# MecatronicaUSB/uwimageproc

Hardware: NVIDIA B200
Metric: chain_frames_per_s_4k (higher is better)
Workload: dtype u8 (histretch, aclahe) / int32+f64 (bgdehaze)

## Files before the change

### include/uwip.h

```cpp
#ifndef UWIP_H
#define UWIP_H

#include <stddef.h>
#include <stdint.h>

#ifdef __cplusplus
extern "C" {
#endif

#define UWIP_VERSION 100

typedef enum uwip_status {
  UWIP_OK = 0,
  UWIP_ERR_INVALID = -1,
  UWIP_ERR_CUDA = -2,
  UWIP_ERR_UNSUPPORTED = -3,
  UWIP_ERR_NOMEM = -4
} uwip_status;

typedef enum uwip_hsv_round {
  UWIP_HSV_ROUND_CV2_4_13 = 0,
  UWIP_HSV_ROUND_TRUNC = 1,
  UWIP_HSV_ROUND_RINT = 2
} uwip_hsv_round;

typedef enum uwip_order {
  UWIP_ORDER_INTENDED = 0,
  UWIP_ORDER_LITERAL = 1
} uwip_order;

typedef struct uwip_ctx uwip_ctx;

int uwip_version(void);
int uwip_create(int device, uwip_ctx** out);
void uwip_destroy(uwip_ctx* ctx);
const char* uwip_last_error(const uwip_ctx* ctx);
int uwip_set_stream(uwip_ctx* ctx, void* cuda_stream);
int uwip_synchronize(uwip_ctx* ctx);
int64_t uwip_launch_count(const uwip_ctx* ctx);
int uwip_profile(uwip_ctx* ctx, int enable);
int uwip_profile_read(uwip_ctx* ctx, const char* tag, double* total_ms, int64_t* launches);

int uwip_device_alloc(uwip_ctx* ctx, size_t bytes, void** dptr);
int uwip_device_free(uwip_ctx* ctx, void* dptr);
int uwip_host_alloc(uwip_ctx* ctx, size_t bytes, void** hptr);
int uwip_host_free(uwip_ctx* ctx, void* hptr);
int uwip_copy_h2d(uwip_ctx* ctx, void* dst_dev, const void* src_host, size_t bytes);
int uwip_copy_d2h(uwip_ctx* ctx, void* dst_host, const void* src_dev, size_t bytes);

int uwip_num_channel(char c);
int uwip_num_space(char c);
int uwip_histogram_u8(uwip_ctx* ctx, const uint8_t* plane, int width, int height, size_t pitch,
                      float hist[256]);
int uwip_histogram_u8_dev(uwip_ctx* ctx, const uint8_t* d_plane, int width, int height,
                          float* d_hist);
int uwip_channel_stretch_u8(uwip_ctx* ctx, const uint8_t* src, size_t src_pitch, uint8_t* dst,
                            size_t dst_pitch, int width, int height, int lo, int hi, int* low_bin,
                            int* high_bin);
int uwip_channel_stretch_u8_dev(uwip_ctx* ctx, const uint8_t* d_src, uint8_t* d_dst, int width,
                                int height, int lo, int hi);
int uwip_channel_stretch_u8_dev_pitched(uwip_ctx* ctx, const uint8_t* d_src, size_t src_pitch,
                                        uint8_t* d_dst, size_t dst_pitch, int width, int height, int lo,
                                        int hi);

int uwip_histretch_bgr8(uwip_ctx* ctx, const uint8_t* src, size_t src_pitch, uint8_t* dst,
                        size_t dst_pitch, int width, int height, const char* channels, int lo,
                        int hi, int order, int hsv_round);
int uwip_histretch_bgr8_dev(uwip_ctx* ctx, const uint8_t* d_src, uint8_t* d_dst, int n_frames,
                            int width, int height, const char* channels, int lo, int hi, int order,
                            int hsv_round);

int uwip_clahe_u8(uwip_ctx* ctx, const uint8_t* src, size_t src_pitch, uint8_t* dst,
                  size_t dst_pitch, int width, int height, double clip, int tiles_x, int tiles_y);
int uwip_clahe_u8_dev(uwip_ctx* ctx, const uint8_t* d_src, uint8_t* d_dst, int n_planes, int width,
                      int height, double clip, int tiles_x, int tiles_y);
int uwip_entropy_u8(uwip_ctx* ctx, const uint8_t* plane, int width, int height, size_t pitch,
                    int flavour, float* entropy);
int uwip_gaussian_blur3_u8(uwip_ctx* ctx, const uint8_t* src, size_t src_pitch, uint8_t* dst,
                           size_t dst_pitch, int width, int height);
int uwip_clahe_entropy_sweep_u8(uwip_ctx* ctx, const uint8_t* plane, int width, int height,
                                size_t pitch, int tiles, const double* clips, int n_clips,
                                int flavour, float* entropies);
int uwip_clahe_entropy_sweep_u8_dev(uwip_ctx* ctx, const uint8_t* d_planes, int n_frames, int width, int height,
                                    const int* grids, int n_grids, const double* clips, int n_clips,
                                    int flavour, float* entropies);
int uwip_aclahe_bgr8(uwip_ctx* ctx, const uint8_t* src, size_t src_pitch, uint8_t* dst,
                     size_t dst_pitch, int width, int height, double clip, int tiles_x,
                     int tiles_y, int hsv_round);
int uwip_aclahe_bgr8_dev(uwip_ctx* ctx, const uint8_t* d_src, uint8_t* d_dst, int n_frames,
                         int width, int height, double clip, int tiles_x, int tiles_y,
                         int hsv_round);

typedef enum uwip_aclahe_loop {
  UWIP_ACLAHE_LOOP_REPAIRED = 0,
  UWIP_ACLAHE_LOOP_AS_COMMITTED = 1
} uwip_aclahe_loop;
int uwip_aclahe_params_u8_dev(uwip_ctx* ctx, const uint8_t* d_planes, int n_planes, int width, int height, int loop,
                              int32_t* d_bs, int32_t* d_cl);
int uwip_aclahe_bgr8_auto_dev(uwip_ctx* ctx, const uint8_t* d_src, uint8_t* d_dst, int n_frames, int width, int height,
                              int loop, int hsv_round, double clip, int tiles_x, int tiles_y, int32_t* d_bs,
                              int32_t* d_cl);

typedef struct uwip_dehaze_params {
  int window;
  int radius;
  double eps;
  double tmin;
} uwip_dehaze_params;
void uwip_dehaze_defaults(uwip_dehaze_params* p);

int uwip_boxfilter_f64(uwip_ctx* ctx, const double* src, int width, int height, int r, double* dst);
int uwip_guided_filter_u8(uwip_ctx* ctx, const uint8_t* guide, size_t pitch, int width, int height,
                          int range, const double* p, int r, double eps, double* q);
int uwip_background_light_bgr8(uwip_ctx* ctx, const uint8_t* src, size_t pitch, int width,
                               int height, int window, double B[3], int64_t idx[2]);
int uwip_transmission_bgr8(uwip_ctx* ctx, const uint8_t* src, size_t pitch, int width, int height,
                           int window, double* t_blue, double* t_green);
int uwip_refined_transmission_bgr8(uwip_ctx* ctx, const uint8_t* src, size_t pitch, int width,
                                   int height, const uwip_dehaze_params* p, double* t_blue,
                                   double* t_green);
int uwip_rc_correction_bgr8(uwip_ctx* ctx, const uint8_t* src, size_t pitch, int width, int height,
                            const uwip_dehaze_params* p, double* restored);
int uwip_bgdehaze_bgr8(uwip_ctx* ctx, const uint8_t* src, size_t src_pitch, uint8_t* dst8,
                       size_t dst_pitch, int width, int height, const uwip_dehaze_params* p,
                       double* out_f64);
int uwip_bgdehaze_bgr8_dev(uwip_ctx* ctx, const uint8_t* d_src, uint8_t* d_dst, int n_frames,
                           int width, int height, const uwip_dehaze_params* p);

typedef struct uwip_chain_params {
  char channels[16];
  int lo, hi;
  int order;
  int hsv_round;
  double clip;
  int tiles_x, tiles_y;
  uwip_dehaze_params dehaze;
} uwip_chain_params;
void uwip_chain_defaults(uwip_chain_params* p);

int uwip_chain_bgr8_dev(uwip_ctx* ctx, const uint8_t* d_src, uint8_t* d_dst, int n_frames,
                        int width, int height, const uwip_chain_params* p);
int uwip_chain_bgr8_auto_dev(uwip_ctx* ctx, const uint8_t* d_src, uint8_t* d_dst, int n_frames, int width, int height,
                             const uwip_chain_params* p, int loop, int32_t* d_bs, int32_t* d_cl);
int uwip_chain_bgr8(uwip_ctx* ctx, const uint8_t* src, uint8_t* dst, int n_frames, int width,
                    int height, const uwip_chain_params* p);

#define UWIP_FRAME_NAN 1
#define UWIP_FRAME_ACLAHE_NOFIT 2
int uwip_last_frame_flags(uwip_ctx* ctx, int n_frames, int32_t* flags_host);

int uwip_calc_blur_bgr8(uwip_ctx* ctx, const uint8_t* src, size_t pitch, int width, int height,
                        int aperture, float* stdev, double* mean_std, uint8_t* lap, size_t lap_pitch);
int uwip_calc_blur_bgr8_dev(uwip_ctx* ctx, const uint8_t* d_src, int n_frames, int width, int height,
                            int aperture, double* d_mean_std);

int uwip_jpeg_info(uwip_ctx* ctx, const uint8_t* jpeg, size_t len, int* width, int* height);
int uwip_jpeg_decode_bgr8_dev(uwip_ctx* ctx, const uint8_t* jpeg, size_t len, uint8_t* d_bgr, int width,
                              int height);
int uwip_jpeg_encode_bgr8_dev(uwip_ctx* ctx, const uint8_t* d_bgr, int width, int height, int quality,
                              uint8_t* out, size_t cap, size_t* out_len);
int uwip_chain_jpeg(uwip_ctx* ctx, const uint8_t* jpeg_in, size_t len_in, const uwip_chain_params* p,
                    int quality, uint8_t* jpeg_out, size_t cap, size_t* len_out);
size_t uwip_jpeg_encode_bound(int width, int height);
int uwip_jpeg_encode_bgr8_batch_dev(uwip_ctx* ctx, const uint8_t* d_bgr, int n_frames, int width, int height, int quality,
                                    uint8_t* d_out, size_t out_stride, uint64_t* d_len);

int uwip_synth_bgr8_dev(uwip_ctx* ctx, uint8_t* d_dst, uint32_t seed, int first_frame, int n_frames,
                        int width, int height);
int uwip_checksum_bgr8_dev(uwip_ctx* ctx, const uint8_t* d_src, int n_frames, int width, int height,
                           uint64_t* sums_host);

#ifdef __cplusplus
}
#endif
#endif
```

### uwimageproc_b200/_lib.py

```python
import ctypes as C
import os

HERE = os.path.dirname(os.path.abspath(__file__))
LIB_PATH = os.path.join(HERE, "libuwip.so")

UWIP_OK = 0


class UwipError(RuntimeError):
    def __init__(self, status, text):
        super().__init__("uwip status %d: %s" % (status, text))
        self.status = status


class DehazeParams(C.Structure):
    _fields_ = [("window", C.c_int), ("radius", C.c_int), ("eps", C.c_double), ("tmin", C.c_double)]


class ChainParams(C.Structure):
    _fields_ = [
        ("channels", C.c_char * 16),
        ("lo", C.c_int), ("hi", C.c_int), ("order", C.c_int), ("hsv_round", C.c_int),
        ("clip", C.c_double), ("tiles_x", C.c_int), ("tiles_y", C.c_int),
        ("dehaze", DehazeParams),
    ]


_P = C.c_void_p
_u8p = C.c_void_p
_sz = C.c_size_t
_i = C.c_int
_d = C.c_double

SIGNATURES = {
    "uwip_version": (_i, []),
    "uwip_create": (_i, [_i, C.POINTER(_P)]),
    "uwip_destroy": (None, [_P]),
    "uwip_last_error": (C.c_char_p, [_P]),
    "uwip_set_stream": (_i, [_P, _P]),
    "uwip_synchronize": (_i, [_P]),
    "uwip_launch_count": (C.c_int64, [_P]),
    "uwip_profile": (_i, [_P, _i]),
    "uwip_profile_read": (_i, [_P, C.c_char_p, C.POINTER(_d), C.POINTER(C.c_int64)]),
    "uwip_device_alloc": (_i, [_P, _sz, C.POINTER(_P)]),
    "uwip_device_free": (_i, [_P, _P]),
    "uwip_host_alloc": (_i, [_P, _sz, C.POINTER(_P)]),
    "uwip_host_free": (_i, [_P, _P]),
    "uwip_copy_h2d": (_i, [_P, _P, _P, _sz]),
    "uwip_copy_d2h": (_i, [_P, _P, _P, _sz]),
    "uwip_num_channel": (_i, [C.c_char]),
    "uwip_num_space": (_i, [C.c_char]),
    "uwip_histogram_u8": (_i, [_P, _u8p, _i, _i, _sz, _P]),
    "uwip_histogram_u8_dev": (_i, [_P, _u8p, _i, _i, _P]),
    "uwip_channel_stretch_u8": (_i, [_P, _u8p, _sz, _u8p, _sz, _i, _i, _i, _i, C.POINTER(_i), C.POINTER(_i)]),
    "uwip_channel_stretch_u8_dev": (_i, [_P, _u8p, _u8p, _i, _i, _i, _i]),
    "uwip_channel_stretch_u8_dev_pitched": (_i, [_P, _u8p, _sz, _u8p, _sz, _i, _i, _i, _i]),
    "uwip_histretch_bgr8": (_i, [_P, _u8p, _sz, _u8p, _sz, _i, _i, C.c_char_p, _i, _i, _i, _i]),
    "uwip_histretch_bgr8_dev": (_i, [_P, _u8p, _u8p, _i, _i, _i, C.c_char_p, _i, _i, _i, _i]),
    "uwip_clahe_u8": (_i, [_P, _u8p, _sz, _u8p, _sz, _i, _i, _d, _i, _i]),
    "uwip_clahe_u8_dev": (_i, [_P, _u8p, _u8p, _i, _i, _i, _d, _i, _i]),
    "uwip_entropy_u8": (_i, [_P, _u8p, _i, _i, _sz, _i, C.POINTER(C.c_float)]),
    "uwip_gaussian_blur3_u8": (_i, [_P, _u8p, _sz, _u8p, _sz, _i, _i]),
    "uwip_clahe_entropy_sweep_u8": (_i, [_P, _u8p, _i, _i, _sz, _i, C.POINTER(_d), _i, _i, C.POINTER(C.c_float)]),
    "uwip_clahe_entropy_sweep_u8_dev": (_i, [_P, _u8p, _i, _i, _i, C.POINTER(_i), _i, C.POINTER(_d), _i, _i, C.POINTER(C.c_float)]),
    "uwip_aclahe_bgr8": (_i, [_P, _u8p, _sz, _u8p, _sz, _i, _i, _d, _i, _i, _i]),
    "uwip_aclahe_bgr8_dev": (_i, [_P, _u8p, _u8p, _i, _i, _i, _d, _i, _i, _i]),
    "uwip_aclahe_params_u8_dev": (_i, [_P, _u8p, _i, _i, _i, _i, _P, _P]),
    "uwip_aclahe_bgr8_auto_dev": (_i, [_P, _u8p, _u8p, _i, _i, _i, _i, _i, _d, _i, _i, _P, _P]),
    "uwip_dehaze_defaults": (None, [C.POINTER(DehazeParams)]),
    "uwip_chain_defaults": (None, [C.POINTER(ChainParams)]),
    "uwip_boxfilter_f64": (_i, [_P, _P, _i, _i, _i, _P]),
    "uwip_guided_filter_u8": (_i, [_P, _u8p, _sz, _i, _i, _i, _P, _i, _d, _P]),
    "uwip_background_light_bgr8": (_i, [_P, _u8p, _sz, _i, _i, _i, C.POINTER(_d), C.POINTER(C.c_int64)]),
    "uwip_transmission_bgr8": (_i, [_P, _u8p, _sz, _i, _i, _i, _P, _P]),
    "uwip_refined_transmission_bgr8": (_i, [_P, _u8p, _sz, _i, _i, C.POINTER(DehazeParams), _P, _P]),
    "uwip_rc_correction_bgr8": (_i, [_P, _u8p, _sz, _i, _i, C.POINTER(DehazeParams), _P]),
    "uwip_bgdehaze_bgr8": (_i, [_P, _u8p, _sz, _u8p, _sz, _i, _i, C.POINTER(DehazeParams), _P]),
    "uwip_bgdehaze_bgr8_dev": (_i, [_P, _u8p, _u8p, _i, _i, _i, C.POINTER(DehazeParams)]),
    "uwip_chain_bgr8_dev": (_i, [_P, _u8p, _u8p, _i, _i, _i, C.POINTER(ChainParams)]),
    "uwip_chain_bgr8_auto_dev": (_i, [_P, _u8p, _u8p, _i, _i, _i, C.POINTER(ChainParams), _i, _P, _P]),
    "uwip_chain_bgr8": (_i, [_P, _u8p, _u8p, _i, _i, _i, C.POINTER(ChainParams)]),
    "uwip_last_frame_flags": (_i, [_P, _i, _P]),
    "uwip_jpeg_info": (_i, [_P, _u8p, _sz, C.POINTER(_i), C.POINTER(_i)]),
    "uwip_jpeg_decode_bgr8_dev": (_i, [_P, _u8p, _sz, _u8p, _i, _i]),
    "uwip_jpeg_encode_bgr8_dev": (_i, [_P, _u8p, _i, _i, _i, _u8p, _sz, C.POINTER(_sz)]),
    "uwip_chain_jpeg": (_i, [_P, _u8p, _sz, C.POINTER(ChainParams), _i, _u8p, _sz, C.POINTER(_sz)]),
    "uwip_jpeg_encode_bound": (_sz, [_i, _i]),
    "uwip_jpeg_encode_bgr8_batch_dev": (_i, [_P, _u8p, _i, _i, _i, _i, _u8p, _sz, _P]),
    "uwip_calc_blur_bgr8": (_i, [_P, _u8p, _sz, _i, _i, _i, C.POINTER(C.c_float), C.POINTER(_d), _u8p, _sz]),
    "uwip_calc_blur_bgr8_dev": (_i, [_P, _u8p, _i, _i, _i, _i, _P]),
    "uwip_synth_bgr8_dev": (_i, [_P, _u8p, C.c_uint32, _i, _i, _i, _i]),
    "uwip_checksum_bgr8_dev": (_i, [_P, _u8p, _i, _i, _i, _P]),
}

_lib = None


def load():
    global _lib
    if _lib is not None:
        return _lib
    if not os.path.exists(LIB_PATH):
        raise UwipError(-2, "libuwip.so is not built: run `python -c 'import __graft_entry__ as g; g.build()'` "
                            "(nvcc, sm_100a).  There is no CPU fallback.")
    lib = C.CDLL(LIB_PATH)
    for name, (res, args) in SIGNATURES.items():
        fn = getattr(lib, name)
        fn.restype = res
        fn.argtypes = args
    _lib = lib
    return lib
```

### uwimageproc_b200/csrc/cabi.cu

```cuda
#include <stdarg.h>

#include <algorithm>
#include <mutex>

#include "common.cuh"
#include "e2e_schedule.h"

struct DeviceGuard {
  int prev = -1;
  explicit DeviceGuard(int dev) {
    if (cudaGetDevice(&prev) != cudaSuccess) prev = -1;
    if (prev != dev) cudaSetDevice(dev); else prev = -1;
  }
  ~DeviceGuard() { if (prev >= 0) cudaSetDevice(prev); }
};
static thread_local std::string g_create_err;

const char* uwip_set_err(uwip_ctx* ctx, const char* fmt, ...) {
  char buf[1024];
  va_list ap;
  va_start(ap, fmt);
  vsnprintf(buf, sizeof(buf), fmt, ap);
  va_end(ap);
  if (ctx) ctx->err = buf; else g_create_err = buf;
// ... 255 lines not shown
  UWIP_REQUIRE(ctx, d_src && d_dst && w > 0 && h > 0, "bad argument");
  UWIP_CHECK(check_percentiles(ctx, lo, hi));
  uint32_t* dh = (uint32_t*)uwip_slot(ctx, SLOT_HIST, 256 * 4);
  uint8_t* dl = (uint8_t*)uwip_slot(ctx, SLOT_LUT, 1024);
  FrameState* fs = frame_state_get(ctx, 1);
  if (!dh || !dl || !fs) return UWIP_ERR_NOMEM;
  UWIP_CHECK(k_histogram_plane(ctx, d_src, 1, (size_t)w * h, dh));
  UWIP_CHECK(k_percentile_lut(ctx, dh, 1, w, h, lo, hi, fs, dl));
  return k_apply_lut_plane(ctx, d_src, d_dst, 1, (size_t)w * h, dl);
}

int uwip_channel_stretch_u8_dev_pitched(uwip_ctx* ctx, const uint8_t* d_src, size_t src_pitch, uint8_t* d_dst, size_t dst_pitch, int w, int h,
                                        int lo, int hi) {
  CTX_GUARD(ctx);
  UWIP_REQUIRE(ctx, d_src && d_dst && w > 0 && h > 0 && src_pitch >= (size_t)w && dst_pitch >= (size_t)w, "bad argument");
  if (src_pitch == (size_t)w && dst_pitch == (size_t)w) return uwip_channel_stretch_u8_dev(ctx, d_src, d_dst, w, h, lo, hi);
  uint8_t* tmp = (uint8_t*)uwip_slot(ctx, SLOT_STAGE_IN, (size_t)w * h);
  if (!tmp) return UWIP_ERR_NOMEM;
  UWIP_CUDA(ctx, cudaMemcpy2DAsync(tmp, (size_t)w, d_src, src_pitch, (size_t)w, (size_t)h, cudaMemcpyDeviceToDevice, ctx->stream));
  UWIP_CHECK(uwip_channel_stretch_u8_dev(ctx, tmp, tmp, w, h, lo, hi));
  UWIP_CUDA(ctx, cudaMemcpy2DAsync(d_dst, dst_pitch, tmp, (size_t)w, (size_t)w, (size_t)h, cudaMemcpyDeviceToDevice, ctx->stream));
  return UWIP_OK;
}

int uwip_channel_stretch_u8(uwip_ctx* ctx, const uint8_t* src, size_t sp, uint8_t* dst, size_t dp, int w, int h, int lo, int hi,
                            int* low_bin, int* high_bin) {
  CTX_GUARD(ctx);
  uint8_t* d;
  UWIP_CHECK(stage_in(ctx, SLOT_STAGE_IN, src, sp, w, h, 1, &d));
  UWIP_CHECK(uwip_channel_stretch_u8_dev(ctx, d, d, w, h, lo, hi));
  if (low_bin || high_bin) {
    FrameState* hs = (FrameState*)ctx->pinned;
    UWIP_CUDA(ctx, cudaMemcpyAsync(hs, frame_state_get(ctx, 1), sizeof(FrameState), cudaMemcpyDeviceToHost, ctx->stream));
    UWIP_CUDA(ctx, cudaStreamSynchronize(ctx->stream));
    if (low_bin) *low_bin = hs->low;
    if (high_bin) *high_bin = hs->high;
  }
  return stage_out(ctx, d, dst, dp, w, h, 1);
}

int uwip_histretch_bgr8_dev(uwip_ctx* ctx, const uint8_t* d_src, uint8_t* d_dst, int n, int w, int h, const char* channels, int lo,
                            int hi, int order, int hsv_round) {
  CTX_GUARD(ctx);
  UWIP_REQUIRE(ctx, d_src && d_dst && channels && n > 0 && w > 0 && h > 0, "bad argument");
  UWIP_REQUIRE(ctx, order == 0 || order == 1, "order must be 0 (intended) or 1 (literal)");
  UWIP_REQUIRE(ctx, hsv_round >= 0 && hsv_round <= 2, "bad hsv_round");
  UWIP_CHECK(check_percentiles(ctx, lo, hi));
  return histretch_frames_dev(ctx, d_src, d_dst, n, w, h, channels, lo, hi, order, hsv_round);
}
int uwip_histretch_bgr8(uwip_ctx* ctx, const uint8_t* src, size_t sp, uint8_t* dst, size_t dp, int w, int h, const char* channels,
                        int lo, int hi, int order, int hsv_round) {
  CTX_GUARD(ctx);
  uint8_t* d;
  UWIP_CHECK(stage_in(ctx, SLOT_STAGE_IN, src, sp, w, h, 3, &d));
  UWIP_CHECK(uwip_histretch_bgr8_dev(ctx, d, d, 1, w, h, channels, lo, hi, order, hsv_round));
  return stage_out(ctx, d, dst, dp, w, h, 3);
}

int uwip_clahe_u8_dev(uwip_ctx* ctx, const uint8_t* d_src, uint8_t* d_dst, int n, int w, int h, double clip, int tx, int ty) {
  CTX_GUARD(ctx);
  UWIP_REQUIRE(ctx, d_src && d_dst, "null pointer");
  return clahe_planes_dev(ctx, d_src, d_dst, n, w, h, clip, tx, ty);
}
int uwip_clahe_u8(uwip_ctx* ctx, const uint8_t* src, size_t sp, uint8_t* dst, size_t dp, int w, int h, double clip, int tx, int ty) {
  CTX_GUARD(ctx);
  uint8_t* d;
  UWIP_CHECK(stage_in(ctx, SLOT_STAGE_IN, src, sp, w, h, 1, &d));
  uint8_t* o = (uint8_t*)uwip_slot(ctx, SLOT_STAGE_OUT, (size_t)w * h);
  if (!o) return UWIP_ERR_NOMEM;
  UWIP_CHECK(clahe_planes_dev(ctx, d, o, 1, w, h, clip, tx, ty));
  return stage_out(ctx, o, dst, dp, w, h, 1);
}
int uwip_entropy_u8(uwip_ctx* ctx, const uint8_t* plane, int w, int h, size_t pitch, int flavour, float* entropy) {
  CTX_GUARD(ctx);
  UWIP_REQUIRE(ctx, entropy && (flavour == 0 || flavour == 1), "bad argument");
  uint8_t* d;
  UWIP_CHECK(stage_in(ctx, SLOT_STAGE_IN, plane, pitch, w, h, 1, &d));
  uint32_t* dh = (uint32_t*)uwip_slot(ctx, SLOT_HIST, 256 * 4);
  float* de = (float*)uwip_slot(ctx, SLOT_MISC, 256);
  if (!dh || !de) return UWIP_ERR_NOMEM;
  UWIP_CHECK(k_histogram_plane(ctx, d, 1, (size_t)w * h, dh));
  UWIP_CHECK(k_entropy(ctx, dh, 1, w, h, flavour, de));
  UWIP_CUDA(ctx, cudaMemcpyAsync(entropy, de, 4, cudaMemcpyDeviceToHost, ctx->stream));
  UWIP_CUDA(ctx, cudaStreamSynchronize(ctx->stream));
  return UWIP_OK;
}
int uwip_gaussian_blur3_u8(uwip_ctx* ctx, const uint8_t* src, size_t sp, uint8_t* dst, size_t dp, int w, int h) {
  CTX_GUARD(ctx);
  uint8_t* d;
  UWIP_CHECK(stage_in(ctx, SLOT_STAGE_IN, src, sp, w, h, 1, &d));
  uint8_t* o = (uint8_t*)uwip_slot(ctx, SLOT_STAGE_OUT, (size_t)w * h);
  if (!o) return UWIP_ERR_NOMEM;
  UWIP_CHECK(k_blur3(ctx, d, o, w, h));
  return stage_out(ctx, o, dst, dp, w, h, 1);
}
int uwip_clahe_entropy_sweep_u8(uwip_ctx* ctx, const uint8_t* plane, int w, int h, size_t pitch, int tiles, const double* clips,
                                int n_clips, int flavour, float* entropies) {
  CTX_GUARD(ctx);
  UWIP_REQUIRE(ctx, clips && entropies && (flavour == 0 || flavour == 1), "bad argument");
  uint8_t* d;
  UWIP_CHECK(stage_in(ctx, SLOT_STAGE_IN, plane, pitch, w, h, 1, &d));
  return clahe_entropy_sweep_dev(ctx, d, w, h, tiles, clips, n_clips, flavour, entropies);
}
int uwip_clahe_entropy_sweep_u8_dev(uwip_ctx* ctx, const uint8_t* d_planes, int n, int w, int h, const int* grids, int n_grids,
                                    const double* clips, int n_clips, int flavour, float* entropies) {
  CTX_GUARD(ctx);
  UWIP_REQUIRE(ctx, d_planes && grids && clips && entropies && (flavour == 0 || flavour == 1), "bad argument");
  return clahe_entropy_sweep_batch_dev(ctx, d_planes, n, w, h, grids, n_grids, clips, n_clips, flavour, entropies);
}
int uwip_aclahe_bgr8_dev(uwip_ctx* ctx, const uint8_t* d_src, uint8_t* d_dst, int n, int w, int h, double clip, int tx, int ty,
                         int hsv_round) {
  CTX_GUARD(ctx);
  UWIP_REQUIRE(ctx, d_src && d_dst && hsv_round >= 0 && hsv_round <= 2, "bad argument");
  return aclahe_frames_dev(ctx, d_src, d_dst, n, w, h, clip, tx, ty, hsv_round, nullptr, nullptr);
}
int uwip_aclahe_bgr8(uwip_ctx* ctx, const uint8_t* src, size_t sp, uint8_t* dst, size_t dp, int w, int h, double clip, int tx, int ty,
                     int hsv_round) {
  CTX_GUARD(ctx);
  uint8_t* d;
  UWIP_CHECK(stage_in(ctx, SLOT_STAGE_IN, src, sp, w, h, 3, &d));
  UWIP_CHECK(uwip_aclahe_bgr8_dev(ctx, d, d, 1, w, h, clip, tx, ty, hsv_round));
  return stage_out(ctx, d, dst, dp, w, h, 3);
}

static int32_t* flags_get(uwip_ctx* ctx, int n);

static int auto_outputs(uwip_ctx* ctx, int n, int32_t*& d_bs, int32_t*& d_cl) {
  if (d_bs && d_cl) return UWIP_OK;
  int32_t* ws = (int32_t*)uwip_slot(ctx, SLOT_AUTO_BSCL, sizeof(int32_t) * 2 * (size_t)n);
  if (!ws) return UWIP_ERR_NOMEM;
  if (!d_bs) d_bs = ws;
  if (!d_cl) d_cl = ws + n;
  return UWIP_OK;
}

int uwip_aclahe_params_u8_dev(uwip_ctx* ctx, const uint8_t* d_planes, int n, int w, int h, int loop, int32_t* d_bs, int32_t* d_cl) {
  CTX_GUARD(ctx);
  UWIP_REQUIRE(ctx, d_planes && d_bs && d_cl && n > 0 && w > 0 && h > 0, "bad argument");
  int32_t* flags = flags_get(ctx, n);
  if (!flags) return UWIP_ERR_NOMEM;
  UWIP_CHECK(aclahe_params_planes_dev(ctx, d_planes, n, w, h, loop, d_bs, d_cl));
  return aclahe_nofit_flags(ctx, d_cl, n, flags, false);
}
int uwip_aclahe_bgr8_auto_dev(uwip_ctx* ctx, const uint8_t* d_src, uint8_t* d_dst, int n, int w, int h, int loop, int hsv_round,
                              double clip, int tx, int ty, int32_t* d_bs, int32_t* d_cl) {
  CTX_GUARD(ctx);
  UWIP_REQUIRE(ctx, d_src && d_dst && n > 0 && w > 0 && h > 0 && hsv_round >= 0 && hsv_round <= 2, "bad argument");
  UWIP_CHECK(auto_outputs(ctx, n, d_bs, d_cl));
  int32_t* flags = flags_get(ctx, n);
  if (!flags) return UWIP_ERR_NOMEM;
  UWIP_CHECK(aclahe_frames_auto_dev(ctx, d_src, d_dst, n, w, h, loop, clip, tx, ty, hsv_round, nullptr, nullptr, d_bs, d_cl));
  return aclahe_nofit_flags(ctx, d_cl, n, flags, false);
}

int uwip_calc_blur_bgr8_dev(uwip_ctx* ctx, const uint8_t* d_src, int n, int w, int h, int aperture, double* d_mean_std) {
  CTX_GUARD(ctx);
  UWIP_REQUIRE(ctx, d_src && d_mean_std && n >= 1 && w >= 1 && h >= 1 && (aperture == 1 || aperture == 3), "bad argument");
  return calc_blur_frames_dev(ctx, d_src, n, w, h, aperture, d_mean_std, nullptr);
}
int uwip_calc_blur_bgr8(uwip_ctx* ctx, const uint8_t* src, size_t pitch, int w, int h, int aperture, float* stdev, double* mean_std,
                        uint8_t* lap, size_t lap_pitch) {
  CTX_GUARD(ctx);
  UWIP_REQUIRE(ctx, stdev || mean_std || lap, "no output requested");
  UWIP_REQUIRE(ctx, aperture == 1 || aperture == 3, "aperture must be 1 or 3");
  uint8_t* d;
  UWIP_CHECK(stage_in(ctx, SLOT_STAGE_IN, src, pitch, w, h, 3, &d));
  double* d_out = (double*)uwip_slot(ctx, SLOT_BLUROUT, 16);
  uint8_t* d_lap = lap ? (uint8_t*)uwip_slot(ctx, SLOT_STAGE_OUT, (size_t)w * h) : nullptr;
  if (!d_out || (lap && !d_lap)) return UWIP_ERR_NOMEM;
  UWIP_CHECK(calc_blur_frames_dev(ctx, d, 1, w, h, aperture, d_out, d_lap));
  double ms[2];
  UWIP_CUDA(ctx, cudaMemcpyAsync(ms, d_out, 16, cudaMemcpyDeviceToHost, ctx->stream));
  if (lap) UWIP_CHECK(stage_out(ctx, d_lap, lap, lap_pitch, w, h, 1));
  UWIP_CUDA(ctx, cudaStreamSynchronize(ctx->stream));
  if (stdev) *stdev = (float)ms[1];
  if (mean_std) { mean_std[0] = ms[0]; mean_std[1] = ms[1]; }
  return UWIP_OK;
}

void uwip_dehaze_defaults(uwip_dehaze_params* p) {
  if (!p) return;
  p->window = 15; p->radius = 40; p->eps = 1e-3; p->tmin = 0.2;
}
void uwip_chain_defaults(uwip_chain_params* p) {
  if (!p) return;
  memset(p, 0, sizeof(*p));
  strcpy(p->channels, "V");
  p->lo = 1; p->hi = 99; p->order = UWIP_ORDER_INTENDED; p->hsv_round = UWIP_HSV_ROUND_CV2_4_13;
  p->clip = 2.0; p->tiles_x = 8; p->tiles_y = 8;
  uwip_dehaze_defaults(&p->dehaze);
}

static int dehaze_host(uwip_ctx* ctx, const uint8_t* src, size_t pitch, int w, int h, const uwip_dehaze_params* pp, int stop_after,
                       uint8_t* dst8, size_t dst_pitch, double B[3], int64_t idx[2], double* t_raw, double* t_ref, double* restored,
                       double* out) {
  uwip_dehaze_params p;
  if (pp) p = *pp; else uwip_dehaze_defaults(&p);
  uint8_t* d;
  UWIP_CHECK(stage_in(ctx, SLOT_STAGE_IN, src, pitch, w, h, 3, &d));
  size_t n_px = (size_t)w * h;
  uint8_t* o = (uint8_t*)uwip_slot(ctx, SLOT_STAGE_OUT, n_px * 3);
  double* f64 = (double*)uwip_slot(ctx, SLOT_F64OUT, n_px * 8 * 8);
  FrameState* fs = frame_state_get(ctx, 1);
  if (!o || !f64 || !fs) return UWIP_ERR_NOMEM;
  DehazeDebug dbg;
  dbg.t_raw = t_raw ? f64 : nullptr;
  dbg.t_ref = t_ref ? f64 + 2 * n_px : nullptr;
  dbg.restored = restored ? f64 + 4 * n_px : nullptr;
  dbg.out = out ? f64 + 4 * n_px : nullptr;
  dbg.stop_after = stop_after;
  UWIP_CHECK(frame_state_reset(ctx, fs, 1));
  UWIP_CHECK(dehaze_frames_dev(ctx, d, o, 1, w, h, p, false, fs, &dbg));
  FrameState* hs = (FrameState*)ctx->pinned;
  UWIP_CUDA(ctx, cudaMemcpyAsync(hs, fs, sizeof(FrameState), cudaMemcpyDeviceToHost, ctx->stream));
  if (t_raw) UWIP_CUDA(ctx, cudaMemcpyAsync(t_raw, dbg.t_raw, 2 * n_px * 8, cudaMemcpyDeviceToHost, ctx->stream));
  if (t_ref) UWIP_CUDA(ctx, cudaMemcpyAsync(t_ref, dbg.t_ref, 2 * n_px * 8, cudaMemcpyDeviceToHost, ctx->stream));
  if (restored) UWIP_CUDA(ctx, cudaMemcpyAsync(restored, dbg.restored, 3 * n_px * 8, cudaMemcpyDeviceToHost, ctx->stream));
  if (out) UWIP_CUDA(ctx, cudaMemcpyAsync(out, dbg.out, 3 * n_px * 8, cudaMemcpyDeviceToHost, ctx->stream));
  UWIP_CUDA(ctx, cudaStreamSynchronize(ctx->stream));
  if (B) { B[0] = hs->B[0]; B[1] = hs->B[1]; B[2] = hs->B[2]; }
  if (idx) { idx[0] = hs->idx0; idx[1] = hs->idx1; }
  if (dst8) return stage_out(ctx, o, dst8, dst_pitch, w, h, 3);
  return UWIP_OK;
}

int uwip_background_light_bgr8(uwip_ctx* ctx, const uint8_t* src, size_t pitch, int w, int h, int window, double B[3], int64_t idx[2]) {
  CTX_GUARD(ctx);
  uwip_dehaze_params p;
  uwip_dehaze_defaults(&p);
  p.window = window;
  return dehaze_host(ctx, src, pitch, w, h, &p, 1, nullptr, 0, B, idx, nullptr, nullptr, nullptr, nullptr);
}
int uwip_transmission_bgr8(uwip_ctx* ctx, const uint8_t* src, size_t pitch, int w, int h, int window, double* t_blue, double* t_green) {
  CTX_GUARD(ctx);
  UWIP_REQUIRE(ctx, t_blue && t_green, "null output");
  UWIP_REQUIRE(ctx, window == 15, "transmission window other than 15 is not reachable in the reference chain (BGDehaze.py:52)");
  uwip_dehaze_params p;
  uwip_dehaze_defaults(&p);
  size_t n_px = (size_t)w * h;
  std::vector<double> tmp(2 * n_px);
  UWIP_CHECK(dehaze_host(ctx, src, pitch, w, h, &p, 2, nullptr, 0, nullptr, nullptr, tmp.data(), nullptr, nullptr, nullptr));
  memcpy(t_blue, tmp.data(), n_px * 8);
  memcpy(t_green, tmp.data() + n_px, n_px * 8);
  return UWIP_OK;
}
int uwip_refined_transmission_bgr8(uwip_ctx* ctx, const uint8_t* src, size_t pitch, int w, int h, const uwip_dehaze_params* p,
                                   double* t_blue, double* t_green) {
  CTX_GUARD(ctx);
  UWIP_REQUIRE(ctx, t_blue && t_green, "null output");
  size_t n_px = (size_t)w * h;
  std::vector<double> tmp(2 * n_px);
  UWIP_CHECK(dehaze_host(ctx, src, pitch, w, h, p, 3, nullptr, 0, nullptr, nullptr, nullptr, tmp.data(), nullptr, nullptr));
  memcpy(t_blue, tmp.data(), n_px * 8);
  memcpy(t_green, tmp.data() + n_px, n_px * 8);
  return UWIP_OK;
}
int uwip_rc_correction_bgr8(uwip_ctx* ctx, const uint8_t* src, size_t pitch, int w, int h, const uwip_dehaze_params* p, double* restored) {
  CTX_GUARD(ctx);
  UWIP_REQUIRE(ctx, restored, "null output");
  return dehaze_host(ctx, src, pitch, w, h, p, 4, nullptr, 0, nullptr, nullptr, nullptr, nullptr, restored, nullptr);
}
int uwip_bgdehaze_bgr8(uwip_ctx* ctx, const uint8_t* src, size_t sp, uint8_t* dst8, size_t dp, int w, int h, const uwip_dehaze_params* p,
                       double* out_f64) {
  CTX_GUARD(ctx);
  UWIP_REQUIRE(ctx, dst8, "null output");
  return dehaze_host(ctx, src, sp, w, h, p, 0, dst8, dp, nullptr, nullptr, nullptr, nullptr, nullptr, out_f64);
}

int uwip_boxfilter_f64(uwip_ctx* ctx, const double* src, int w, int h, int r, double* dst) {
  CTX_GUARD(ctx);
  UWIP_REQUIRE(ctx, src && dst && w >= 1 && h >= 1 && r >= 0, "bad argument");
  const size_t n_px = (size_t)w * h;
  double* d = (double*)uwip_slot(ctx, SLOT_F64OUT, n_px * 8 * 3);
  if (!d) return UWIP_ERR_NOMEM;
  UWIP_CUDA(ctx, cudaMemcpyAsync(d, src, n_px * 8, cudaMemcpyHostToDevice, ctx->stream));
  UWIP_CHECK(boxfilter_f64_dev(ctx, d, d + n_px, d + 2 * n_px, w, h, r));
  UWIP_CUDA(ctx, cudaMemcpyAsync(dst, d + 2 * n_px, n_px * 8, cudaMemcpyDeviceToHost, ctx->stream));
  UWIP_CUDA(ctx, cudaStreamSynchronize(ctx->stream));
  return UWIP_OK;
}
int uwip_guided_filter_u8(uwip_ctx* ctx, const uint8_t* guide, size_t pitch, int w, int h, int range, const double* p, int r, double eps,
                          double* q) {
  CTX_GUARD(ctx);
  UWIP_REQUIRE(ctx, guide && p && q, "null argument");
  uint8_t* d_g;
  UWIP_CHECK(stage_in(ctx, SLOT_STAGE_IN, guide, pitch, w, h, 3, &d_g));
  const size_t n_px = (size_t)w * h;
  double* d = (double*)uwip_slot(ctx, SLOT_F64OUT, n_px * 8 * 2);
  FrameState* fs = frame_state_get(ctx, 1);
  if (!d || !fs) return UWIP_ERR_NOMEM;
  UWIP_CUDA(ctx, cudaMemcpyAsync(d, p, n_px * 8, cudaMemcpyHostToDevice, ctx->stream));
  UWIP_CHECK(guided_filter_u8_dev(ctx, d_g, d, d + n_px, w, h, range, r, eps, fs));
  FrameState* hs = (FrameState*)ctx->pinned;
  UWIP_CUDA(ctx, cudaMemcpyAsync(hs, fs, sizeof(FrameState), cudaMemcpyDeviceToHost, ctx->stream));
  UWIP_CUDA(ctx, cudaMemcpyAsync(q, d + n_px, n_px * 8, cudaMemcpyDeviceToHost, ctx->stream));
  UWIP_CUDA(ctx, cudaStreamSynchronize(ctx->stream));
  if (hs->nan_flag & 2u) {
    uwip_set_err(ctx, "uwip_guided_filter_u8: p must lie in [0, 1.6] (the signals of the path do: transmission <= 1, exposure ratio <= 1.54)");
    return UWIP_ERR_INVALID;
  }
  return UWIP_OK;
}

static int32_t* flags_get(uwip_ctx* ctx, int n) {
  int32_t* f = (int32_t*)uwip_slot(ctx, SLOT_FLAGS, sizeof(int32_t) * (size_t)n);
  ctx->flags_n = f ? n : 0;
  return f;
}

static int sub_batch(const uwip_ctx* ctx, int n, int w, int h) {
  size_t per_frame = (size_t)w * h * 60 + (512u << 10);
  double gb = 80.0;
  if (const char* e = getenv("UWIP_WORKSPACE_GB")) { double v = atof(e); if (v >= 1.0) gb = v; }
  size_t cap_bytes = (size_t)(gb * 1e9);
  size_t free_b = 0, total_b = 0;
  if (cudaMemGetInfo(&free_b, &total_b) == cudaSuccess) {
    size_t held = 0;
    for (int i = 0; i < uwip_ctx::kSlots; i++) held += ctx->slot_bytes[i];
    cap_bytes = std::min(cap_bytes, (size_t)(0.7 * (double)(free_b + held)));
  } else {
    cudaGetLastError();
  }
  size_t cap = std::max<size_t>(1, cap_bytes / per_frame);
  return dehaze_sub_batch(ctx, n, w, (int)std::min<size_t>(cap, (size_t)n));
}

int uwip_bgdehaze_bgr8_dev(uwip_ctx* ctx, const uint8_t* d_src, uint8_t* d_dst, int n, int w, int h, const uwip_dehaze_params* pp) {
  CTX_GUARD(ctx);
  UWIP_REQUIRE(ctx, d_src && d_dst && n > 0, "bad argument");
  uwip_dehaze_params p;
  if (pp) p = *pp; else uwip_dehaze_defaults(&p);
  int nb = sub_batch(ctx, n, w, h);
  FrameState* fs = frame_state_get(ctx, nb);
  int32_t* flags = flags_get(ctx, n);
  if (!fs || !flags) return UWIP_ERR_NOMEM;
  size_t fbytes = (size_t)w * h * 3;
  for (int i = 0; i < n; i += nb) {
    int m = std::min(nb, n - i);
    UWIP_CHECK(frame_state_reset(ctx, fs, m));
    UWIP_CHECK(dehaze_frames_dev(ctx, d_src + (size_t)i * fbytes, d_dst + (size_t)i * fbytes, m, w, h, p, false, fs, nullptr, flags + i));
  }
  return UWIP_OK;
}

struct ChainAuto {
  int loop;
  int32_t* d_bs;
  int32_t* d_cl;
};

static int chain_aclahe(uwip_ctx* ctx, const uint8_t* d_src, uint8_t* d_dst, int m, int w, int h, const uwip_chain_params& p,
                        const uint8_t* d_prelut, FrameState* fs, const ChainAuto* au) {
  if (au)
    return aclahe_frames_auto_dev(ctx, d_src, d_dst, m, w, h, au->loop, p.clip, p.tiles_x, p.tiles_y, p.hsv_round, d_prelut, fs, au->d_bs,
                                  au->d_cl);
  return aclahe_frames_dev(ctx, d_src, d_dst, m, w, h, p.clip, p.tiles_x, p.tiles_y, p.hsv_round, d_prelut, fs);
}

static int chain_sub(uwip_ctx* ctx, const uint8_t* d_src, uint8_t* d_dst, int m, int w, int h, const uwip_chain_params& p, FrameState* fs, int32_t* flags,
                     const ChainAuto* au = nullptr) {
  size_t fbytes = (size_t)w * h * 3;
  uint8_t* tmp = (uint8_t*)uwip_slot(ctx, SLOT_TMP_FRAME, fbytes * m);
  if (!tmp) return UWIP_ERR_NOMEM;
  UWIP_CHECK(frame_state_reset(ctx, fs, m));
  bool fused_head = (strcmp(p.channels, "V") == 0 && p.order == UWIP_ORDER_INTENDED);
  if (fused_head) {
    uint32_t* d_hist = (uint32_t*)uwip_slot(ctx, SLOT_HIST, (size_t)m * 256 * 4);
    uint8_t* d_lut = (uint8_t*)uwip_slot(ctx, SLOT_LUT, (size_t)m * 256 * 4);
    if (!d_hist || !d_lut) return UWIP_ERR_NOMEM;
    UWIP_CHECK(k_histogram_frame(ctx, d_src, m, w, h, CH_V, d_hist));
    UWIP_CHECK(k_percentile_lut(ctx, d_hist, m, w, h, p.lo, p.hi, fs, d_lut));
    UWIP_CHECK(chain_aclahe(ctx, d_src, tmp, m, w, h, p, d_lut, fs, au));
  } else {
    UWIP_CHECK(histretch_frames_dev(ctx, d_src, tmp, m, w, h, p.channels, p.lo, p.hi, p.order, p.hsv_round));
    UWIP_CHECK(chain_aclahe(ctx, tmp, tmp, m, w, h, p, nullptr, fs, au));
  }
  UWIP_CHECK(dehaze_frames_dev(ctx, tmp, d_dst, m, w, h, p.dehaze, true, fs, nullptr, flags));
  return au ? aclahe_nofit_flags(ctx, au->d_cl, m, flags, true) : UWIP_OK;
}

static int chain_reserve(uwip_ctx* ctx, int m, int w, int h, const uwip_chain_params& p) {
  const size_t fbytes = (size_t)w * h * 3, n_pp = (size_t)((w + 3) & ~3) * h;
  const size_t ntile = (size_t)m * std::max(1, p.tiles_x) * std::max(1, p.tiles_y);
  const struct { int slot; size_t bytes; } want[] = {
      {SLOT_TMP_FRAME, fbytes * m}, {SLOT_HIST, (size_t)m * 256 * 4}, {SLOT_LUT, (size_t)m * 256 * 4},
      {SLOT_TILEHIST, ntile * 256 * 4}, {SLOT_TILELUT, ntile * 256 + 16}, {SLOT_MISC, 256},
      {SLOT_KQ, m * n_pp * 4}, {SLOT_MPLANES, m * n_pp}, {SLOT_YCC, m * n_pp * 4}, {SLOT_STAB, (size_t)m * 65536 * 8},
      {SLOT_SPLANE, m * n_pp * 4}, {SLOT_AB, m * n_pp * 32}, {SLOT_J, m * n_pp * 8}, {SLOT_REFS, m * n_pp * 4}};
  for (const auto& e : want)
    if (!uwip_slot(ctx, e.slot, e.bytes)) return UWIP_ERR_NOMEM;
  return UWIP_OK;
}

static int chain_check(uwip_ctx* ctx, const uwip_chain_params* p, int n, int w, int h) {
  UWIP_REQUIRE(ctx, p, "null params (use uwip_chain_defaults)");
  UWIP_REQUIRE(ctx, n > 0 && w > 0 && h > 0, "bad size");
  UWIP_REQUIRE(ctx, memchr(p->channels, 0, sizeof(p->channels)) != nullptr, "channels not terminated");
  UWIP_REQUIRE(ctx, p->order == 0 || p->order == 1, "bad order");
  UWIP_REQUIRE(ctx, p->hsv_round >= 0 && p->hsv_round <= 2, "bad hsv_round");
  return check_percentiles(ctx, p->lo, p->hi);
}

int uwip_chain_bgr8_dev(uwip_ctx* ctx, const uint8_t* d_src, uint8_t* d_dst, int n, int w, int h, const uwip_chain_params* p) {
  CTX_GUARD(ctx);
  UWIP_REQUIRE(ctx, d_src && d_dst, "null pointer");
  UWIP_CHECK(chain_check(ctx, p, n, w, h));
  int nb = sub_batch(ctx, n, w, h);
  FrameState* fs = frame_state_get(ctx, nb);
  int32_t* flags = flags_get(ctx, n);
  if (!fs || !flags) return UWIP_ERR_NOMEM;
  size_t fbytes = (size_t)w * h * 3;
  for (int i = 0; i < n; i += nb) {
    int m = std::min(nb, n - i);
    UWIP_CHECK(chain_sub(ctx, d_src + (size_t)i * fbytes, d_dst + (size_t)i * fbytes, m, w, h, *p, fs, flags + i));
  }
  return UWIP_OK;
}

int uwip_chain_bgr8_auto_dev(uwip_ctx* ctx, const uint8_t* d_src, uint8_t* d_dst, int n, int w, int h, const uwip_chain_params* p, int loop,
                             int32_t* d_bs, int32_t* d_cl) {
  CTX_GUARD(ctx);
  UWIP_REQUIRE(ctx, d_src && d_dst, "null pointer");
  UWIP_CHECK(chain_check(ctx, p, n, w, h));
  UWIP_REQUIRE(ctx, loop == UWIP_ACLAHE_LOOP_REPAIRED || loop == UWIP_ACLAHE_LOOP_AS_COMMITTED, "bad loop");
  UWIP_CHECK(aclahe_check_auto_size(ctx, w, h));
  UWIP_CHECK(auto_outputs(ctx, n, d_bs, d_cl));
  int nb = sub_batch(ctx, n, w, h);
  FrameState* fs = frame_state_get(ctx, nb);
  int32_t* flags = flags_get(ctx, n);
  if (!fs || !flags) return UWIP_ERR_NOMEM;
  size_t fbytes = (size_t)w * h * 3;
  for (int i = 0; i < n; i += nb) {
    int m = std::min(nb, n - i);
    ChainAuto au = {loop, d_bs + i, d_cl + i};
    UWIP_CHECK(chain_sub(ctx, d_src + (size_t)i * fbytes, d_dst + (size_t)i * fbytes, m, w, h, *p, fs, flags + i, &au));
  }
  return UWIP_OK;
}

int uwip_chain_bgr8(uwip_ctx* ctx, const uint8_t* src, uint8_t* dst, int n, int w, int h, const uwip_chain_params* p) {
  CTX_GUARD(ctx);
  UWIP_REQUIRE(ctx, src && dst, "null pointer");
  UWIP_CHECK(chain_check(ctx, p, n, w, h));
  int nb = sub_batch(ctx, n, w, h);
  nb = std::max(1, std::min(nb, (n + 1) / 2));
  std::vector<int> sizes = e2e_schedule(n, nb, ctx->sm_count, dehaze_strips(w), dehaze_strips_narrow(w));
  if (const char* e = getenv("UWIP_E2E_SIZES")) {
    std::vector<int> v;
    long sum = 0;
    for (const char* q = e; *q;) {
      char* end = nullptr;
      long m = strtol(q, &end, 10);
      if (end == q || m <= 0) { v.clear(); break; }
      v.push_back((int)m); sum += m;
      q = (*end == ',') ? end + 1 : end;
      if (*end && *end != ',') { v.clear(); break; }
    }
    if (!v.empty() && sum == n && *std::max_element(v.begin(), v.end()) <= nb) sizes = v;
  }
  nb = *std::max_element(sizes.begin(), sizes.end());
  FrameState* fs = frame_state_get(ctx, nb);
  int32_t* flags = flags_get(ctx, n);
  size_t fbytes = (size_t)w * h * 3;
  uint8_t* din[2] = {(uint8_t*)uwip_slot(ctx, SLOT_CHAIN_IN0, fbytes * nb), (uint8_t*)uwip_slot(ctx, SLOT_CHAIN_IN1, fbytes * nb)};
  uint8_t* dout[2] = {(uint8_t*)uwip_slot(ctx, SLOT_CHAIN_OUT0, fbytes * nb), (uint8_t*)uwip_slot(ctx, SLOT_CHAIN_OUT1, fbytes * nb)};
  if (!fs || !flags || !din[0] || !din[1] || !dout[0] || !dout[1]) return UWIP_ERR_NOMEM;
  if (!ctx->s_in) UWIP_CUDA(ctx, cudaStreamCreateWithFlags(&ctx->s_in, cudaStreamNonBlocking));
  if (!ctx->s_out) UWIP_CUDA(ctx, cudaStreamCreateWithFlags(&ctx->s_out, cudaStreamNonBlocking));
  cudaStream_t s_in = ctx->s_in, s_out = ctx->s_out;
  int nsub = (int)sizes.size();
  while ((int)ctx->ev_pool.size() < 3 * nsub + 1) {
    cudaEvent_t e;
    UWIP_CUDA(ctx, cudaEventCreateWithFlags(&e, cudaEventDisableTiming));
    ctx->ev_pool.push_back(e);
  }
  cudaEvent_t* ev_in = ctx->ev_pool.data();
  cudaEvent_t* ev_comp = ev_in + nsub;
  cudaEvent_t* ev_out = ev_comp + nsub;
  cudaEvent_t ev_start = ctx->ev_pool[3 * nsub];
  UWIP_CHECK(chain_reserve(ctx, nb, w, h, *p));
  int rc = UWIP_OK;
  cudaEventRecord(ev_start, ctx->stream);
  cudaStreamWaitEvent(s_in, ev_start, 0);
  size_t first = 0;
  for (int i = 0; i < nsub && rc == UWIP_OK; i++) {
    int m = sizes[i];
    int b = i & 1;
    if (i >= 2) cudaStreamWaitEvent(s_in, ev_comp[i - 2], 0);
    cudaMemcpyAsync(din[b], src + first * fbytes, fbytes * m, cudaMemcpyHostToDevice, s_in);
    cudaEventRecord(ev_in[i], s_in);
    cudaStreamWaitEvent(ctx->stream, ev_in[i], 0);
    if (i >= 2) cudaStreamWaitEvent(ctx->stream, ev_out[i - 2], 0);
    rc = chain_sub(ctx, din[b], dout[b], m, w, h, *p, fs, flags + first);
    cudaEventRecord(ev_comp[i], ctx->stream);
    cudaStreamWaitEvent(s_out, ev_comp[i], 0);
    cudaMemcpyAsync(dst + first * fbytes, dout[b], fbytes * m, cudaMemcpyDeviceToHost, s_out);
    cudaEventRecord(ev_out[i], s_out);
    first += (size_t)m;
  }
  cudaError_t e1 = cudaStreamSynchronize(s_in), e2 = cudaStreamSynchronize(ctx->stream), e3 = cudaStreamSynchronize(s_out);
  if (rc != UWIP_OK) return rc;
  cudaError_t e = e1 != cudaSuccess ? e1 : (e2 != cudaSuccess ? e2 : e3);
  if (e != cudaSuccess) { uwip_set_err(ctx, "chain pipeline: %s", cudaGetErrorString(e)); return UWIP_ERR_CUDA; }
  return UWIP_OK;
}

int uwip_jpeg_info(uwip_ctx* ctx, const uint8_t* jpeg, size_t len, int* width, int* height) {
  CTX_GUARD(ctx);
  UWIP_REQUIRE(ctx, jpeg && len > 0 && width && height, "bad argument");
  return jpeg_info(ctx, jpeg, len, width, height);
}
int uwip_jpeg_decode_bgr8_dev(uwip_ctx* ctx, const uint8_t* jpeg, size_t len, uint8_t* d_bgr, int width, int height) {
  CTX_GUARD(ctx);
  UWIP_REQUIRE(ctx, jpeg && len > 0 && d_bgr && width > 0 && height > 0, "bad argument");
  int w = 0, h = 0;
  UWIP_CHECK(jpeg_info(ctx, jpeg, len, &w, &h));
  UWIP_REQUIRE(ctx, w == width && h == height, "the JPEG stream has another size (uwip_jpeg_info)");
  return jpeg_decode_dev(ctx, jpeg, len, d_bgr, w, h);
}
int uwip_jpeg_encode_bgr8_dev(uwip_ctx* ctx, const uint8_t* d_bgr, int width, int height, int quality, uint8_t* out, size_t cap, size_t* out_len) {
  CTX_GUARD(ctx);
  UWIP_REQUIRE(ctx, d_bgr && width > 0 && height > 0 && out_len && quality >= 1 && quality <= 100, "bad argument");
  return jpeg_encode_dev(ctx, d_bgr, width, height, quality, out, cap, out_len);
}
int uwip_chain_jpeg(uwip_ctx* ctx, const uint8_t* jpeg_in, size_t len_in, const uwip_chain_params* p, int quality, uint8_t* jpeg_out,
                    size_t cap, size_t* len_out) {
  CTX_GUARD(ctx);
  UWIP_REQUIRE(ctx, jpeg_in && len_in > 0 && len_out, "bad argument");
  int w = 0, h = 0;
  UWIP_CHECK(jpeg_info(ctx, jpeg_in, len_in, &w, &h));
  UWIP_CHECK(chain_check(ctx, p, 1, w, h));
  const size_t fbytes = (size_t)w * h * 3;
  uint8_t* d_in = (uint8_t*)uwip_slot(ctx, SLOT_CHAIN_IN0, fbytes);
  uint8_t* d_out = (uint8_t*)uwip_slot(ctx, SLOT_CHAIN_OUT0, fbytes);
  FrameState* fs = frame_state_get(ctx, 1);
  int32_t* flags = flags_get(ctx, 1);
  if (!d_in || !d_out || !fs || !flags) return UWIP_ERR_NOMEM;
  UWIP_CHECK(jpeg_decode_dev(ctx, jpeg_in, len_in, d_in, w, h));
  UWIP_CHECK(chain_sub(ctx, d_in, d_out, 1, w, h, *p, fs, flags));
  return jpeg_encode_dev(ctx, d_out, w, h, quality, jpeg_out, cap, len_out);
}

size_t uwip_jpeg_encode_bound(int width, int height) {
  if (width < 1 || width > 65535 || height < 1 || height > 65535) return 0;
  return jpeg_encode_bound(width, height);
}
int uwip_jpeg_encode_bgr8_batch_dev(uwip_ctx* ctx, const uint8_t* d_bgr, int n_frames, int width, int height, int quality, uint8_t* d_out,
                                    size_t out_stride, uint64_t* d_len) {
  CTX_GUARD(ctx);
  UWIP_REQUIRE(ctx, d_bgr && d_out && d_len && n_frames > 0, "bad argument");
  UWIP_REQUIRE(ctx, width >= 1 && width <= 65535 && height >= 1 && height <= 65535, "width and height must lie in 1..65535");
  UWIP_REQUIRE(ctx, quality >= 1 && quality <= 100, "quality must lie in 1..100");
  UWIP_REQUIRE(ctx, out_stride >= jpeg_encode_bound(width, height), "out_stride is below uwip_jpeg_encode_bound(width, height)");
  return jpeg_encode_batch_dev(ctx, d_bgr, n_frames, width, height, quality, d_out, out_stride, d_len);
}

int uwip_last_frame_flags(uwip_ctx* ctx, int n, int32_t* flags_host) {
  CTX_GUARD(ctx);
  UWIP_REQUIRE(ctx, flags_host && n > 0, "bad argument");
  UWIP_REQUIRE(ctx, n <= ctx->flags_n, "more frames requested than the last batched call processed");
  UWIP_CUDA(ctx, cudaMemcpyAsync(flags_host, ctx->slot_ptr[SLOT_FLAGS], sizeof(int32_t) * (size_t)n, cudaMemcpyDeviceToHost, ctx->stream));
  UWIP_CUDA(ctx, cudaStreamSynchronize(ctx->stream));
  return UWIP_OK;
}

int uwip_synth_bgr8_dev(uwip_ctx* ctx, uint8_t* d_dst, uint32_t seed, int first, int n, int w, int h) {
  CTX_GUARD(ctx);
  UWIP_REQUIRE(ctx, d_dst && n > 0 && w > 0 && h > 0 && first >= 0, "bad argument");
  return synth_frames_dev(ctx, d_dst, seed, first, n, w, h);
}
int uwip_checksum_bgr8_dev(uwip_ctx* ctx, const uint8_t* d_src, int n, int w, int h, uint64_t* sums_host) {
  CTX_GUARD(ctx);
  UWIP_REQUIRE(ctx, d_src && sums_host && n > 0, "bad argument");
  return checksum_frames_dev(ctx, d_src, n, w, h, sums_host);
}

}
```

### uwimageproc_b200/csrc/common.cuh

```cuda
#pragma once
#include <cuda_runtime.h>
#include <stdint.h>
#include <stdio.h>
#include <string.h>

#include <string>
#include <vector>

#include "../../include/uwip.h"

struct ProfRec {
  const char* tag;
  cudaEvent_t e0, e1;
};

struct uwip_ctx {
  int device = 0;
  cudaStream_t stream = nullptr;
  bool own_stream = false;
  int sm_count = 148;
  int64_t launches = 0;
  bool profiling = false;
  std::vector<ProfRec> prof;
  std::vector<cudaEvent_t> ev_pool;
  cudaStream_t s_in = nullptr, s_out = nullptr;
  std::string err;
  static const int kSlots = 32;
  void* slot_ptr[kSlots] = {};
  size_t slot_bytes[kSlots] = {};
  void* pinned = nullptr;
  size_t pinned_bytes = 0;
  int flags_n = 0;
  void* jpeg = nullptr;
  static const int kFuncs = 16;
  size_t func_smem[kFuncs] = {};
};

enum FuncId { FUNC_GF1A = 0, FUNC_GF1B, FUNC_GF2A, FUNC_GF2B, FUNC_WINDOW, FUNC_WINDOW15, FUNC_SWEEP, FUNC_GFQ };

template <class K>
static inline cudaError_t uwip_func_smem(uwip_ctx* ctx, int id, K kern, size_t bytes) {
  if (bytes <= ctx->func_smem[id]) return cudaSuccess;
  cudaError_t e = cudaFuncSetAttribute(kern, cudaFuncAttributeMaxDynamicSharedMemorySize, (int)bytes);
  if (e == cudaSuccess) ctx->func_smem[id] = bytes;
  return e;
}

enum Slot {
  SLOT_STAGE_IN = 0,
  SLOT_STAGE_OUT,
  SLOT_HIST,
  SLOT_LUT,
  SLOT_TILEHIST,
  SLOT_TILELUT,
  SLOT_FSTATE,
  SLOT_TMP_FRAME,
  SLOT_MPLANES,
  SLOT_PARTIALS,
  SLOT_AB,
  SLOT_J,
  SLOT_REFS,
  SLOT_F64OUT,
  SLOT_MISC,
  SLOT_CHAIN_IN0,
  SLOT_CHAIN_IN1,
  SLOT_CHAIN_OUT0,
  SLOT_CHAIN_OUT1,
  SLOT_SWEEP,
  SLOT_FLAGS,
  SLOT_KQ,
  SLOT_YCC,
  SLOT_STAB,
  SLOT_SPLANE,
  SLOT_BLURSUMS,
  SLOT_BLUROUT,
  SLOT_APLANE,
  SLOT_ABLUR,
  SLOT_AUTO,
  SLOT_AUTO_BSCL,
  SLOT_JPEGENC,
};

const char* uwip_set_err(uwip_ctx* ctx, const char* fmt, ...);
void* uwip_slot(uwip_ctx* ctx, int slot, size_t bytes);
void uwip_pre_launch(uwip_ctx* ctx, const char* tag);
int uwip_post_launch(uwip_ctx* ctx, const char* tag);

#define UWIP_CUDA(ctx, call)                                                                \
  do {                                                                                      \
    cudaError_t e__ = (call);                                                               \
    if (e__ != cudaSuccess) {                                                               \
      uwip_set_err((ctx), "%s:%d %s -> %s", __FILE__, __LINE__, #call, cudaGetErrorString(e__)); \
      return UWIP_ERR_CUDA;                                                                 \
    }                                                                                       \
  } while (0)

#define UWIP_LAUNCH(ctx, tag, kern, grid, block, smem, ...)            \
  do {                                                                 \
    uwip_pre_launch((ctx), (tag));                                     \
    kern<<<(grid), (block), (smem), (ctx)->stream>>>(__VA_ARGS__);     \
    int rc__ = uwip_post_launch((ctx), (tag));                         \
    if (rc__ != UWIP_OK) return rc__;                                  \
  } while (0)

#define UWIP_CHECK(expr)          \
  do {                            \
    int rc__ = (expr);            \
    if (rc__ != UWIP_OK) return rc__; \
  } while (0)

#define UWIP_REQUIRE(ctx, cond, msg)                       \
  do {                                                     \
    if (!(cond)) {                                         \
      uwip_set_err((ctx), "%s: %s", __func__, (msg));      \
      return UWIP_ERR_INVALID;                             \
    }                                                      \
  } while (0)

static inline int cdiv(int a, int b) { return (a + b - 1) / b; }
static inline size_t align_up(size_t x, size_t a) { return (x + a - 1) / a * a; }

struct FrameState {
  int low, high;
  unsigned int kmin, kmax;
  unsigned int idx0, idx1;
  double B[3];
  double Bt[3];
  unsigned long long jmin_key[2], jmax_key[2];
  long long jsum_fix[2];
  unsigned int rmin, rmax;
  unsigned long long rsum;
  unsigned int yi_min, yi_max, yj_min, yj_max;
  unsigned long long omin_key, omax_key;
  unsigned int nan_flag;
  unsigned int pad;
};

__host__ __device__ inline unsigned long long dkey(double d) {
  unsigned long long u;
#ifdef __CUDA_ARCH__
  u = (unsigned long long)__double_as_longlong(d);
#else
  memcpy(&u, &d, 8);
#endif
  return (u & 0x8000000000000000ull) ? ~u : (u | 0x8000000000000000ull);
}
__host__ __device__ inline double dunkey(unsigned long long k) {
  unsigned long long u = (k & 0x8000000000000000ull) ? (k & 0x7fffffffffffffffull) : ~k;
#ifdef __CUDA_ARCH__
  return __longlong_as_double((long long)u);
#else
  double d;
  memcpy(&d, &u, 8);
  return d;
#endif
}

__device__ __forceinline__ int hsv_sdiv(int i) { return i ? ((255 << 12) * 2 + i) / (2 * i) : 0; }
__device__ __forceinline__ int hsv_hdiv(int i) { return i ? (2 * 122880 + i) / (2 * i) : 0; }

enum Channel {
  CH_B = 0, CH_G = 1, CH_R = 2, CH_H = 3, CH_S = 4, CH_V = 5, CH_Y = 6, CH_CR = 7, CH_CB = 8,
  CH_HLS_H = 9, CH_HLS_L = 10, CH_HLS_S = 11,
  CH_LAB_L = 12, CH_LAB_A = 13, CH_LAB_B = 14
};

__device__ __forceinline__ int imax3(int a, int b, int c) { return max(max(a, b), c); }
__device__ __forceinline__ int imin3(int a, int b, int c) { return min(min(a, b), c); }

__device__ __forceinline__ void bgr2hsv_u8(int b, int g, int r, const int* __restrict__ sdiv,
                                           const int* __restrict__ hdiv, int& h, int& s, int& v) {
  v = imax3(b, g, r);
  int d = v - imin3(b, g, r);
  s = (d * sdiv[v] + (1 << 11)) >> 12;
  int h0 = (v == r) ? (g - b) : ((v == g) ? (b - r + 2 * d) : (r - g + 4 * d));
  h = (h0 * hdiv[d] + (1 << 11)) >> 12;
  if (h < 0) h += 180;
}

__device__ __forceinline__ void hsv2bgr_u8(int H, int S, int V, bool trunc_mode, int& b, int& g,
                                           int& r) {
  const float hscale = 6.0f / 180.0f;
  const float k255 = 1.0f / 255.0f;
  float h = __fmul_rn((float)H, hscale);
  float s = __fmul_rn((float)S, k255);
  float v = __fmul_rn((float)V, k255);
  float fsec = floorf(h);
  float f = __fsub_rn(h, fsec);
  int sec = (int)fsec;
  if ((unsigned)sec >= 6u) {
    sec = 0;
    f = 0.f;
  }
  float t0 = v;
  float t1 = __fmul_rn(v, __fsub_rn(1.0f, s));
  float t2 = __fmul_rn(v, __fmaf_rn(-s, f, 1.0f));
  float t3 = __fmul_rn(v, __fmaf_rn(-s, __fsub_rn(1.0f, f), 1.0f));
  float fb, fg, fr;
  switch (sec) {
    case 0: fb = t1; fg = t3; fr = t0; break;
    case 1: fb = t1; fg = t0; fr = t2; break;
    case 2: fb = t3; fg = t0; fr = t1; break;
    case 3: fb = t0; fg = t2; fr = t1; break;
    case 4: fb = t0; fg = t1; fr = t3; break;
    default: fb = t2; fg = t1; fr = t0; break;
  }
  fb = __fmul_rn(fb, 255.0f);
  fg = __fmul_rn(fg, 255.0f);
  fr = __fmul_rn(fr, 255.0f);
  if (trunc_mode) {
    b = __float2int_rz(fb); g = __float2int_rz(fg); r = __float2int_rz(fr);
  } else {
    b = __float2int_rn(fb); g = __float2int_rn(fg); r = __float2int_rn(fr);
  }
  b = min(max(b, 0), 255);
  g = min(max(g, 0), 255);
  r = min(max(r, 0), 255);
}

__device__ __forceinline__ int hsv_roundtrip_v(int Vn, bool trunc_mode) {
  float v = __fmul_rn(__fmul_rn((float)Vn, 1.0f / 255.0f), 255.0f);
  int o = trunc_mode ? __float2int_rz(v) : __float2int_rn(v);
  return min(max(o, 0), 255);
}

__device__ __forceinline__ void bgr2ycrcb_u8(int b, int g, int r, int& Y, int& Cr, int& Cb) {
  Y = (4899 * r + 9617 * g + 1868 * b + 8192) >> 14;
  Cr = ((r - Y) * 11682 + 128 * 16384 + 8192) >> 14;
  Cb = ((b - Y) * 9241 + 128 * 16384 + 8192) >> 14;
  Cr = min(max(Cr, 0), 255);
  Cb = min(max(Cb, 0), 255);
}

__device__ __forceinline__ void ycrcb2bgr_u8(int Y, int Cr, int Cb, int& b, int& g, int& r) {
  Cr -= 128; Cb -= 128;
  b = Y + ((Cb * 29049 + 8192) >> 14);
  g = Y + ((Cb * -5636 + Cr * -11698 + 8192) >> 14);
  r = Y + ((Cr * 22987 + 8192) >> 14);
  b = min(max(b, 0), 255);
  g = min(max(g, 0), 255);
  r = min(max(r, 0), 255);
}

__device__ __forceinline__ void bgr2hls_u8(int bi, int gi, int ri, bool body, int& H, int& L, int& S) {
  const float k255 = 1.0f / 255.0f;
  float b = __fmul_rn((float)bi, k255), g = __fmul_rn((float)gi, k255), r = __fmul_rn((float)ri, k255);
  float vmax = fmaxf(fmaxf(b, g), r), vmin = fminf(fminf(b, g), r);
  float diff = __fsub_rn(vmax, vmin), vs = __fadd_rn(vmax, vmin);
  float lum = __fmul_rn(vs, 0.5f);
  float hue = 0.f, sat = 0.f;
  if (diff > 1.1920928955078125e-07f) {
    float den = body ? __fsub_rn(2.0f, vs) : __fsub_rn(__fsub_rn(2.0f, vmax), vmin);
    sat = __fdiv_rn(diff, lum < 0.5f ? vs : den);
    float dinv = __fdiv_rn(60.0f, diff);
    float d, add;
    if (vmax == r) { d = __fsub_rn(g, b); add = 0.f; }
    else if (vmax == g) { d = __fsub_rn(b, r); add = 120.f; }
    else { d = __fsub_rn(r, g); add = 240.f; }
    hue = (add == 0.f) ? __fmul_rn(d, dinv) : __fmaf_rn(d, dinv, add);
    if (hue < 0.f) hue = body ? __fmaf_rn(d, dinv, add + 360.f) : __fadd_rn(hue, 360.f);
  }
  H = min(max(__float2int_rn(__fmul_rn(hue, 0.5f)), 0), 255);
  L = min(max(__float2int_rn(__fmul_rn(lum, 255.0f)), 0), 255);
  S = min(max(__float2int_rn(__fmul_rn(sat, 255.0f)), 0), 255);
}

__device__ __forceinline__ void hls2bgr_u8(int H, int L, int S, int& b, int& g, int& r) {
  const float k255 = 1.0f / 255.0f;
  float lum = __fmul_rn((float)L, k255);
  float fb = lum, fg = lum, fr = lum;
  if (S != 0) {
    float s = __fmul_rn((float)S, k255);
    float p2 = (lum <= 0.5f) ? __fmul_rn(lum, __fadd_rn(1.0f, s)) : __fsub_rn(__fadd_rn(lum, s), __fmul_rn(lum, s));
    float p1 = __fsub_rn(__fmul_rn(2.0f, lum), p2);
    float hh = __fmul_rn((float)H, 6.0f / 180.0f);
    float fsec = floorf(hh);
    float f = __fsub_rn(hh, fsec);
    int sec = ((int)fsec) % 6;
    float d = __fsub_rn(p2, p1);
    float t2 = __fadd_rn(p1, __fmul_rn(d, __fsub_rn(1.0f, f)));
    float t3 = __fadd_rn(p1, __fmul_rn(d, f));
    switch (sec) {
      case 0: fb = p1; fg = t3; fr = p2; break;
      case 1: fb = p1; fg = p2; fr = t2; break;
      case 2: fb = t3; fg = p2; fr = p1; break;
      case 3: fb = p2; fg = t2; fr = p1; break;
      case 4: fb = p2; fg = p1; fr = t3; break;
      default: fb = t2; fg = p1; fr = p2; break;
    }
  }
  b = min(max(__float2int_rn(__fmul_rn(fb, 255.0f)), 0), 255);
  g = min(max(__float2int_rn(__fmul_rn(fg, 255.0f)), 0), 255);
  r = min(max(__float2int_rn(__fmul_rn(fr, 255.0f)), 0), 255);
}

__device__ __forceinline__ int sat_rint_u8(float x) {
  if (!(fabsf(x) <= 3.0e9f)) return 0;
  int i = __float2int_rn(x);
  return min(max(i, 0), 255);
}

__device__ __forceinline__ unsigned int warp_reduce_min_u32(unsigned int v) {
  return __reduce_min_sync(0xffffffffu, v);
}
__device__ __forceinline__ unsigned int warp_reduce_max_u32(unsigned int v) {
  return __reduce_max_sync(0xffffffffu, v);
}

int k_histogram_plane(uwip_ctx* ctx, const uint8_t* d_plane, int n_planes, size_t n_px, uint32_t* d_hist);
int calc_blur_frames_dev(uwip_ctx* ctx, const uint8_t* d_src, int n, int w, int h, int aperture, double* d_mean_std, uint8_t* d_lap);
int k_histogram_frame(uwip_ctx* ctx, const uint8_t* d_bgr, int n_frames, int w, int h, int channel, uint32_t* d_hist,
                      int hsv_round = UWIP_HSV_ROUND_CV2_4_13);
int k_percentile_lut(uwip_ctx* ctx, const uint32_t* d_hist, int n, int w, int h, int lo, int hi, FrameState* fs, uint8_t* d_lut);
int k_apply_lut_plane(uwip_ctx* ctx, const uint8_t* d_src, uint8_t* d_dst, int n_planes, size_t n_px, const uint8_t* d_lut);
int k_apply_lut_frame(uwip_ctx* ctx, const uint8_t* d_src, uint8_t* d_dst, int n_frames, int w, int h, int channel, const uint8_t* d_lut, bool use_lut, int hsv_round);
int k_hist_to_float(uwip_ctx* ctx, const uint32_t* d_hist, float* d_out, int n);
int k_entropy(uwip_ctx* ctx, const uint32_t* d_hist, int n_hists, int w, int h, int flavour, float* d_out);
int k_blur3(uwip_ctx* ctx, const uint8_t* d_src, uint8_t* d_dst, int w, int h, int n = 1);
int histretch_frames_dev(uwip_ctx* ctx, const uint8_t* d_src, uint8_t* d_dst, int n, int w, int h, const char* channels, int lo, int hi, int order, int hsv_round);

int clahe_planes_dev(uwip_ctx* ctx, const uint8_t* d_src, uint8_t* d_dst, int n, int w, int h, double clip, int tx, int ty);
int aclahe_frames_dev(uwip_ctx* ctx, const uint8_t* d_src, uint8_t* d_dst, int n, int w, int h, double clip, int tx, int ty, int hsv_round, const uint8_t* d_prelut , FrameState* fs_minmax );
int clahe_entropy_sweep_dev(uwip_ctx* ctx, const uint8_t* d_plane, int w, int h, int tiles, const double* clips, int n_clips, int flavour, float* entropies_host);
int clahe_entropy_sweep_batch_dev(uwip_ctx* ctx, const uint8_t* d_planes, int n, int w, int h, const int* grids, int n_grids, const double* clips, int n_clips, int flavour, float* entropies_host);
int aclahe_check_auto_size(uwip_ctx* ctx, int w, int h);
int aclahe_params_planes_dev(uwip_ctx* ctx, const uint8_t* d_planes, int n, int w, int h, int loop, int* d_bs, int* d_cl);
int aclahe_frames_auto_dev(uwip_ctx* ctx, const uint8_t* d_src, uint8_t* d_dst, int n, int w, int h, int loop, double clip, int tx, int ty, int hsv_round, const uint8_t* d_prelut, FrameState* fs_minmax, int* d_bs, int* d_cl);
int aclahe_nofit_flags(uwip_ctx* ctx, const int* d_cl, int n, int32_t* d_flags, bool keep);

int k_aclahe_knees(uwip_ctx* ctx, const float* d_ent , int n, int n_clips, double* d_xd , int* d_cl);

struct DehazeDebug {
  double* t_raw = nullptr;
  double* t_ref = nullptr;
  double* restored = nullptr;
  double* out = nullptr;
  int stop_after = 0;
};
int dehaze_frames_dev(uwip_ctx* ctx, const uint8_t* d_src, uint8_t* d_dst, int n, int w, int h, const uwip_dehaze_params& p, bool minmax_done, FrameState* fs, DehazeDebug* dbg, int32_t* d_flags = nullptr);
int frame_state_reset(uwip_ctx* ctx, FrameState* fs, int n);
int dehaze_strips(int w);
int dehaze_strips_narrow(int w);
int dehaze_sub_batch(const uwip_ctx* ctx, int n, int w, int cap);
FrameState* frame_state_get(uwip_ctx* ctx, int n);
int boxfilter_f64_dev(uwip_ctx* ctx, const double* d_src, double* d_tmp, double* d_dst, int w, int h, int r);
int guided_filter_u8_dev(uwip_ctx* ctx, const uint8_t* d_guide, const double* d_p, double* d_q, int w, int h, int range, int r, double eps, FrameState* fs);

int jpeg_info(uwip_ctx* ctx, const uint8_t* data, size_t len, int* w, int* h);
int jpeg_decode_dev(uwip_ctx* ctx, const uint8_t* data, size_t len, uint8_t* d_bgr, int w, int h);
int jpeg_encode_dev(uwip_ctx* ctx, const uint8_t* d_bgr, int w, int h, int quality, uint8_t* out, size_t cap, size_t* out_len);
void jpeg_io_destroy(uwip_ctx* ctx);

size_t jpeg_encode_bound(int w, int h);
int jpeg_encode_batch_dev(uwip_ctx* ctx, const uint8_t* d_bgr, int n, int w, int h, int quality, uint8_t* d_out, size_t stride,
                          uint64_t* d_len);

int synth_frames_dev(uwip_ctx* ctx, uint8_t* d_dst, uint32_t seed, int first, int n, int w, int h);
int checksum_frames_dev(uwip_ctx* ctx, const uint8_t* d_src, int n, int w, int h, uint64_t* sums_host);
```

### uwimageproc_b200/csrc/dehaze.cu

```cuda
#include <algorithm>

#include "common.cuh"

__global__ void fs_reset_kernel(FrameState* fs, int n) {
  int i = blockIdx.x * blockDim.x + threadIdx.x;
  if (i >= n) return;
  FrameState s;
  memset(&s, 0, sizeof(s));
  s.kmin = 255; s.kmax = 0;
  s.jmin_key[0] = s.jmin_key[1] = ~0ull;
  s.jmax_key[0] = s.jmax_key[1] = 0ull;
  s.rmin = 255; s.rmax = 0;
  s.yi_min = s.yj_min = 255; s.yi_max = s.yj_max = 0;
  s.omin_key = ~0ull; s.omax_key = 0ull;
  fs[i] = s;
}
int frame_state_reset(uwip_ctx* ctx, FrameState* fs, int n) {
  UWIP_LAUNCH(ctx, "fs_reset", fs_reset_kernel, cdiv(n, 128), 128, 0, fs, n);
  return UWIP_OK;
}
FrameState* frame_state_get(uwip_ctx* ctx, int n) { return (FrameState*)uwip_slot(ctx, SLOT_FSTATE, sizeof(FrameState) * (size_t)n); }

#include "gfmarch.cuh"

// ... 138 lines not shown
}

constexpr int WF_TX = 64, WF_TY = 32, WF_R = 7, WF_RH = WF_TY + 2 * WF_R;
constexpr int WF_VR = WF_TY / 4, WF_CTAS = 3;
constexpr int WF_RB = 8;
constexpr int WF_PP = 84;
constexpr int WF_HP = 68;
constexpr int WF_HN = 16;

template <int N, bool MAX, int OFF, int M>
__device__ __forceinline__ void win15(const uint32_t (&p)[M], uint32_t (&o)[N]) {
  static_assert(OFF + N + 14 <= M, "window run");
  uint32_t a[N + 12], b[N + 6];
#pragma unroll
  for (int i = 0; i < N + 12; i++)
    a[i] = MAX ? __vimax3_u16x2(p[OFF + i], p[OFF + i + 1], p[OFF + i + 2]) : __vimin3_u16x2(p[OFF + i], p[OFF + i + 1], p[OFF + i + 2]);
#pragma unroll
  for (int i = 0; i < N + 6; i++) b[i] = MAX ? __vimax3_u16x2(a[i], a[i + 3], a[i + 6]) : __vimin3_u16x2(a[i], a[i + 3], a[i + 6]);
#pragma unroll
  for (int i = 0; i < N; i++) o[i] = MAX ? __vmaxu2(b[i], b[i + 6]) : __vminu2(b[i], b[i + 6]);
}

__device__ __forceinline__ void wf_cp_async8(void* smem, const void* gmem) {
  asm volatile("cp.async.ca.shared.global [%0], [%1], 8;" ::"r"((uint32_t)__cvta_generic_to_shared(smem)), "l"(gmem) : "memory");
}

template <bool FAST>
__device__ __forceinline__ uint32_t wf_emit_rows(const uint32_t (&mx0)[WF_VR], const uint32_t (&mx1)[WF_VR], const uint32_t (&mn0)[WF_VR],
                                                 const uint32_t* __restrict__ pc0, const uint32_t* __restrict__ pc1,
                                                 uint32_t* __restrict__ kqp, uint8_t* __restrict__ mgq, unsigned Wp, int nrows, int gy0, int H,
                                                 bool xt, bool inside, uint32_t km2) {
  uint32_t dmin2 = 0xffffffffu;
#pragma unroll
  for (int i = 0; i < WF_VR; i++) {
    if (!FAST && i >= nrows) break;
    const unsigned o = (unsigned)i * Wp;
    if (!FAST && !inside) { kqp[o] = 0u; mgq[o] = 0; continue; }
    const uint32_t t0 = pc0[i * WF_PP] - km2, t1 = pc1[i * WF_PP] - km2;
    uint32_t tn = mn0[i] - km2;
    if (!FAST) {
      const int gy = gy0 + i;
      if (xt || gy < WF_R || gy + WF_R >= H) tn = 0u;
    }
    kqp[o] = __byte_perm(__byte_perm(t0, t1, 0x4420), tn, 0x4210);
    mgq[o] = (uint8_t)(tn >> 16);
    dmin2 = __vminu2(dmin2, mx1[i] + 0x01000100u - mx0[i]);
  }
  return dmin2;
}

template <int CH>
__device__ __forceinline__ void wf_exact(const uint32_t (&mx0)[WF_VR], const uint32_t (&mx1)[WF_VR], int nrows, uint32_t target, int kmin,
                                         const double* s_nrm, unsigned idx0, unsigned W, double& bd, unsigned& bi) {
#pragma unroll
  for (int i = 0; i < WF_VR; i++) {
    if (i >= nrows) break;
    const uint32_t mr = mx1[i] & 0xffffu, mc = CH ? (mx0[i] >> 16) : (mx0[i] & 0xffffu);
    if (mr + 256u - mc == target) {
      const double d = s_nrm[mr - kmin] - s_nrm[mc - kmin];
      if (d < bd) { bd = d; bi = idx0 + (unsigned)i * W; }
    }
  }
}

__global__ void __launch_bounds__(256, WF_CTAS) window15_kernel(const uint8_t* __restrict__ src, int W, int H, int Wp,
                                                          const FrameState* __restrict__ fs, uint32_t* __restrict__ kq,
                                                          uint8_t* __restrict__ mgp, ArgPartial* __restrict__ partials) {
  extern __shared__ __align__(16) uint32_t s_w[];
  __shared__ double s_nrm[256];
  __shared__ uint32_t s_wmin[8];
  __shared__ int s_cnt[2];
  uint32_t* P0 = s_w;
  uint32_t* P1 = P0 + WF_RH * WF_PP;
  uint32_t* HX0 = P1 + WF_RH * WF_PP;
  uint32_t* HX1 = HX0 + WF_RH * WF_HP;
  uint32_t* HN0 = HX1 + WF_RH * WF_HP;
  const int f = blockIdx.z, tid = threadIdx.x, lane = tid & 31, warp = tid >> 5;
  const uint8_t* img = src + (size_t)f * W * H * 3;
  const int x0 = blockIdx.x * WF_TX, y0 = blockIdx.y * WF_TY;
  const int kmin = fs[f].kmin, range = (int)fs[f].kmax - kmin;
  s_nrm[tid] = (double)tid / (double)range;
  if (tid < 2) s_cnt[tid] = 0;
  uint32_t* RAW = HX0;
  const bool words = ((W & 3) == 0) && ((reinterpret_cast<uintptr_t>(img) & 3) == 0);
  const bool dwords = ((W & 7) == 0) && ((reinterpret_cast<uintptr_t>(img) & 7) == 0);
  if (dwords && x0 >= WF_RB && x0 - WF_RB + 80 <= W) {
    const uint2* col = reinterpret_cast<const uint2*>(img + (size_t)(x0 - WF_RB) * 3);
#pragma unroll
    for (int k = 0; k < (WF_RH + 7) / 8; k++) {
      const int ry = warp + 8 * k;
      if (ry < WF_RH && lane < 30) {
        const int y = min(max(y0 - WF_R + ry, 0), H - 1);
        wf_cp_async8(reinterpret_cast<uint2*>(RAW + ry * 64) + lane, col + (size_t)y * (W * 3 / 8) + lane);
      }
    }
    asm volatile("cp.async.wait_all;" ::: "memory");
    __syncthreads();
    for (int t = tid; t < WF_RH * 20; t += 256) {
      const int ry = t / 20, g = t - ry * 20;
      const uint32_t* w = RAW + ry * 64 + 3 * g;
      const uint32_t w0 = w[0], w1 = w[1], w2 = w[2];
      uint4 bg, rr;
      bg.x = __byte_perm(w0, 0u, 0x4140); bg.y = __byte_perm(w0, w1, 0x0403) & 0x00ff00ffu;
      bg.z = __byte_perm(w1, 0u, 0x4342); bg.w = __byte_perm(w2, 0u, 0x4241);
      rr.x = __byte_perm(w0, 0u, 0x4242); rr.y = __byte_perm(w1, 0u, 0x4141);
      rr.z = __byte_perm(w2, 0u, 0x4040); rr.w = __byte_perm(w2, 0u, 0x4343);
      *reinterpret_cast<uint4*>(P0 + ry * WF_PP + 4 * g) = bg;
      *reinterpret_cast<uint4*>(P1 + ry * WF_PP + 4 * g) = rr;
    }
  } else if (words) {
    const int xa = max(x0 - WF_RB, 0), xb = min(x0 - WF_RB + 79, W - 1);
    const int byte0 = (xa * 3) & ~3;
    const int nw = ((xb * 3 + 2) >> 2) - (byte0 >> 2) + 1;
#pragma unroll 4
    for (int idx = tid; idx < WF_RH * 64; idx += 256) {
      const int ry = idx >> 6, wi = idx & 63;
      if (wi < nw) {
        const int y = min(max(y0 - WF_R + ry, 0), H - 1);
        RAW[idx] = __ldg(reinterpret_cast<const uint32_t*>(img + (size_t)y * W * 3 + byte0) + wi);
      }
    }
    __syncthreads();
    if (tid < 240) {
      const int rx = tid % 80, rr = tid / 80;
      const int xc = min(max(x0 - WF_RB + rx, 0), W - 1);
      const uint8_t* rawb = reinterpret_cast<const uint8_t*>(RAW) + (xc * 3 - byte0);
#pragma unroll 7
      for (int ry = rr; ry < WF_RH; ry += 3) {
        const uint8_t* p = rawb + ry * 256;
        uint32_t b = p[0], g = p[1], r = p[2];
        P0[ry * WF_PP + rx] = b | (g << 16);
        P1[ry * WF_PP + rx] = r | (r << 16);
      }
    }
  } else if (tid < 240) {
    const int rx = tid % 80, rr = tid / 80;
    const int xc = min(max(x0 - WF_RB + rx, 0), W - 1);
    const uint8_t* col = img + (size_t)xc * 3;
#pragma unroll 7
    for (int ry = rr; ry < WF_RH; ry += 3) {
      const int y = min(max(y0 - WF_R + ry, 0), H - 1);
      const uint8_t* p = col + (size_t)y * W * 3;
      uint32_t b = __ldg(p), g = __ldg(p + 1), r = __ldg(p + 2);
      P0[ry * WF_PP + rx] = b | (g << 16);
      P1[ry * WF_PP + rx] = r | (r << 16);
    }
  }
  __syncthreads();
  if (tid < WF_RH * (WF_TX / WF_HN)) {
    const int ry = tid % WF_RH, j = tid / WF_RH;
    uint32_t p[WF_HN + 16], o[WF_HN];
    const uint4* r0 = reinterpret_cast<const uint4*>(P0 + ry * WF_PP + WF_HN * j);
#pragma unroll
    for (int q = 0; q < (WF_HN + 16) / 4; q++) { const uint4 v = r0[q]; p[4 * q] = v.x; p[4 * q + 1] = v.y; p[4 * q + 2] = v.z; p[4 * q + 3] = v.w; }
    win15<WF_HN, true, 1>(p, o);
    uint4* h0 = reinterpret_cast<uint4*>(HX0 + ry * WF_HP + WF_HN * j);
#pragma unroll
    for (int q = 0; q < WF_HN / 4; q++) h0[q] = make_uint4(o[4 * q], o[4 * q + 1], o[4 * q + 2], o[4 * q + 3]);
    win15<WF_HN, false, 1>(p, o);
    uint4* hn = reinterpret_cast<uint4*>(HN0 + ry * WF_HP + WF_HN * j);
#pragma unroll
    for (int q = 0; q < WF_HN / 4; q++) hn[q] = make_uint4(o[4 * q], o[4 * q + 1], o[4 * q + 2], o[4 * q + 3]);
    const uint4* r1 = reinterpret_cast<const uint4*>(P1 + ry * WF_PP + WF_HN * j);
#pragma unroll
    for (int q = 0; q < (WF_HN + 16) / 4; q++) { const uint4 v = r1[q]; p[4 * q] = v.x; p[4 * q + 1] = v.y; p[4 * q + 2] = v.z; p[4 * q + 3] = v.w; }
    win15<WF_HN, true, 1>(p, o);
    uint4* h1 = reinterpret_cast<uint4*>(HX1 + ry * WF_HP + WF_HN * j);
#pragma unroll
    for (int q = 0; q < WF_HN / 4; q++) h1[q] = make_uint4(o[4 * q], o[4 * q + 1], o[4 * q + 2], o[4 * q + 3]);
  }
  __syncthreads();
  const int x = tid & 63, run = tid >> 6;
  const int gx = x0 + x, ry0 = run * WF_VR, gy0 = y0 + ry0;
  const int nrows = gx < Wp ? min(WF_VR, H - gy0) : 0;
  const bool inside = gx < W;
  uint32_t mx0[WF_VR], mx1[WF_VR], dmin2 = 0xffffffffu;
  if (nrows > 0) {
    uint32_t p[WF_VR + 14], mn0[WF_VR];
#pragma unroll
    for (int i = 0; i < WF_VR + 14; i++) p[i] = HX0[(ry0 + i) * WF_HP + x];
    win15<WF_VR, true, 0>(p, mx0);
#pragma unroll
    for (int i = 0; i < WF_VR + 14; i++) p[i] = HX1[(ry0 + i) * WF_HP + x];
    win15<WF_VR, true, 0>(p, mx1);
#pragma unroll
    for (int i = 0; i < WF_VR + 14; i++) p[i] = HN0[(ry0 + i) * WF_HP + x];
    win15<WF_VR, false, 0>(p, mn0);
    const size_t pix0 = (size_t)f * Wp * H + (size_t)gy0 * Wp + gx;
    const uint32_t* pc0 = P0 + (ry0 + WF_R) * WF_PP + x + WF_RB;
    const uint32_t* pc1 = P1 + (ry0 + WF_R) * WF_PP + x + WF_RB;
    const uint32_t km2 = (uint32_t)kmin * 0x10001u;
    const bool xt = (gx < WF_R) || (gx + WF_R >= W);
    if (!xt && gy0 >= WF_R && gy0 + WF_VR - 1 + WF_R < H)
      dmin2 = wf_emit_rows<true>(mx0, mx1, mn0, pc0, pc1, kq + pix0, mgp + pix0, (unsigned)Wp, nrows, gy0, H, xt, inside, km2);
    else
      dmin2 = wf_emit_rows<false>(mx0, mx1, mn0, pc0, pc1, kq + pix0, mgp + pix0, (unsigned)Wp, nrows, gy0, H, xt, inside, km2);
  }
  {
    const uint32_t m0 = __reduce_min_sync(0xffffffffu, dmin2 & 0xffffu), m1 = __reduce_min_sync(0xffffffffu, dmin2 >> 16);
    if (lane == 0) s_wmin[warp] = m0 | (m1 << 16);
  }
  __syncthreads();
  double* cand_d = reinterpret_cast<double*>(HX0);
  unsigned* cand_i = reinterpret_cast<unsigned*>(cand_d + 512);
  uint32_t cm2 = s_wmin[0];
#pragma unroll
  for (int k = 1; k < 8; k++) cm2 = __vminu2(cm2, s_wmin[k]);
  if (inside && nrows > 0) {
    const unsigned idx0 = (unsigned)gy0 * (unsigned)W + (unsigned)gx;
    if ((dmin2 & 0xffffu) == (cm2 & 0xffffu)) {
      double bd = __longlong_as_double(0x7ff0000000000000ll); unsigned bi = 0xffffffffu;
      wf_exact<0>(mx0, mx1, nrows, cm2 & 0xffffu, kmin, s_nrm, idx0, (unsigned)W, bd, bi);
      const int slot = atomicAdd(&s_cnt[0], 1);
      cand_d[slot] = bd; cand_i[slot] = bi;
    }
    if ((dmin2 >> 16) == (cm2 >> 16)) {
      double bd = __longlong_as_double(0x7ff0000000000000ll); unsigned bi = 0xffffffffu;
      wf_exact<1>(mx0, mx1, nrows, cm2 >> 16, kmin, s_nrm, idx0, (unsigned)W, bd, bi);
      const int slot = atomicAdd(&s_cnt[1], 1);
      cand_d[256 + slot] = bd; cand_i[256 + slot] = bi;
    }
  }
  __syncthreads();
  if (warp < 2) {
    const int n = s_cnt[warp];
    double bd = __longlong_as_double(0x7ff0000000000000ll); unsigned bi = 0xffffffffu;
    for (int k = lane; k < n; k += 32) {
      const double d = cand_d[warp * 256 + k]; const unsigned i = cand_i[warp * 256 + k];
      if (lex_less(d, i, bd, bi)) { bd = d; bi = i; }
    }
#pragma unroll
    for (int d = 16; d > 0; d >>= 1) {
      const double od = __shfl_xor_sync(0xffffffffu, bd, d); const unsigned oi = __shfl_xor_sync(0xffffffffu, bi, d);
      if (lex_less(od, oi, bd, bi)) { bd = od; bi = oi; }
    }
    if (lane == 0) {
      ArgPartial* a = partials + ((size_t)f * gridDim.x * gridDim.y + blockIdx.y * gridDim.x + blockIdx.x);
      if (bi == 0xffffffffu) bd = __longlong_as_double(0x7ff0000000000000ll);
      if (warp == 0) { a->d0 = bd; a->i0 = bi; } else { a->d1 = bd; a->i1 = bi; }
    }
  }
}

__global__ void __launch_bounds__(256) bglight_finish_kernel(const uint8_t* __restrict__ src, int W, int H,
                                                             const ArgPartial* __restrict__ partials, int n_part, FrameState* fs,
                                                             int write_B, int write_Bt) {
  __shared__ ArgPartial s_part[8];
  int f = blockIdx.x;
  const ArgPartial* pp = partials + (size_t)f * n_part;
  double bd0 = __longlong_as_double(0x7ff0000000000000ll), bd1 = bd0;
  unsigned bi0 = 0xffffffffu, bi1 = 0xffffffffu;
  for (int i = threadIdx.x; i < n_part; i += 256) {
    ArgPartial a = pp[i];
    if (lex_less(a.d0, a.i0, bd0, bi0)) { bd0 = a.d0; bi0 = a.i0; }
    if (lex_less(a.d1, a.i1, bd1, bi1)) { bd1 = a.d1; bi1 = a.i1; }
  }
#pragma unroll
  for (int d = 16; d > 0; d >>= 1) {
    double o0 = __shfl_xor_sync(0xffffffffu, bd0, d), o1 = __shfl_xor_sync(0xffffffffu, bd1, d);
    unsigned j0 = __shfl_xor_sync(0xffffffffu, bi0, d), j1 = __shfl_xor_sync(0xffffffffu, bi1, d);
    if (lex_less(o0, j0, bd0, bi0)) { bd0 = o0; bi0 = j0; }
    if (lex_less(o1, j1, bd1, bi1)) { bd1 = o1; bi1 = j1; }
  }
  if ((threadIdx.x & 31) == 0) { ArgPartial a; a.d0 = bd0; a.d1 = bd1; a.i0 = bi0; a.i1 = bi1; s_part[threadIdx.x >> 5] = a; }
  __syncthreads();
  if (threadIdx.x == 0) {
    ArgPartial a = s_part[0];
    for (int k = 1; k < 8; k++) {
      ArgPartial b = s_part[k];
      if (lex_less(b.d0, b.i0, a.d0, a.i0)) { a.d0 = b.d0; a.i0 = b.i0; }
      if (lex_less(b.d1, b.i1, a.d1, a.i1)) { a.d1 = b.d1; a.i1 = b.i1; }
    }
    FrameState& s = fs[f];
    int kmin = s.kmin;
    double range = (double)((int)s.kmax - kmin);
    if (a.i0 == 0xffffffffu || a.i1 == 0xffffffffu) {
      a.i0 = a.i1 = 0;
      s.nan_flag = 1;
    }
    if (write_B) { s.idx0 = a.i0; s.idx1 = a.i1; }
    const uint8_t* img = src + (size_t)f * W * H * 3;
    for (int c = 0; c < 3; c++) {
      double v0 = (double)((int)img[(size_t)a.i0 * 3 + c] - kmin) / range;
      double v1 = (double)((int)img[(size_t)a.i1 * 3 + c] - kmin) / range;
      double b = (v0 + v1) / 2.0;
      if (write_B) s.B[c] = b;
      if (write_Bt) s.Bt[c] = b;
    }
  }
}

__global__ void traw_kernel(const uint32_t* __restrict__ kq, const uint8_t* __restrict__ mgp, int W, int H, int Wp,
                            const FrameState* __restrict__ fs, double* __restrict__ t_raw) {
  int x = blockIdx.x * blockDim.x + threadIdx.x, y = blockIdx.y;
  if (x >= W) return;
  const FrameState& s = fs[0];
  double range = (double)((int)s.kmax - (int)s.kmin);
  size_t pp = (size_t)y * Wp + x, pix = (size_t)y * W + x;
  int mb = (int)(kq[pp] >> 24), mg = (int)mgp[pp];
  t_raw[pix] = 1.0 - ((double)mb / range) / s.Bt[0];
  t_raw[(size_t)W * H + pix] = 1.0 - ((double)mg / range) / s.Bt[1];
}

constexpr int DZ_ELEMENTWISE_CTAS = 4;
__global__ void __launch_bounds__(256, DZ_ELEMENTWISE_CTAS) exposure_minmax_kernel(GfCommon g, int W, int H, int Wp, double* dbg_restored) {
  __shared__ ExpShared sh;
  int f = blockIdx.y;
  size_t n_pp = (size_t)Wp * H;
  exp_shared_init(&sh, g.fs[f], (double)W * (double)H);
  const uint32_t* kq = g.kq + (size_t)f * n_pp;
  const float* J = g.J + (size_t)f * 2 * n_pp;
  uint32_t* ycc = g.ycc + (size_t)f * n_pp;
  unsigned imn = 255, imx = 0, jmn = 255, jmx = 0;
  const int qpr = Wp / 4;
  const size_t n_q = (size_t)qpr * H;
  for (size_t qi = (size_t)blockIdx.x * 256 + threadIdx.x; qi < n_q; qi += (size_t)gridDim.x * 256) {
    int y = (int)(qi / qpr), x0 = (int)(qi - (size_t)y * qpr) * 4;
    size_t pp = (size_t)y * Wp + x0;
    uint4 kw = __ldg(reinterpret_cast<const uint4*>(kq + pp));
    float4 jb = __ldg(reinterpret_cast<const float4*>(J + pp)), jg = __ldg(reinterpret_cast<const float4*>(J + n_pp + pp));
    uint32_t out[4];
#pragma unroll
    for (int c = 0; c < 4; c++) {
      out[c] = 0;
      if (x0 + c >= W) continue;
      uint32_t w = quad_get(kw, c);
      uint32_t kb = w & 255u, kg = (w >> 8) & 255u, kr = (w >> 16) & 255u;
      int r8b = restored_byte(quad_get(jb, c), sh.fc, 0), r8g = restored_byte(quad_get(jg, c), sh.fc, 1), r8r = sh.rt.red8[kr];
      if (dbg_restored && f == 0) {
        size_t pix = (size_t)y * W + x0 + c;
        dbg_restored[pix * 3] = norm_j(quad_get(jb, c), sh.fc, 0); dbg_restored[pix * 3 + 1] = norm_j(quad_get(jg, c), sh.fc, 1);
        dbg_restored[pix * 3 + 2] = sh.rt.redN[kr];
      }
      int Yi, Cri, Cbi, Yj, Crj, Cbj;
      bgr2ycrcb_u8(sh.rt.i8[kb], sh.rt.i8[kg], sh.rt.i8[kr], Yi, Cri, Cbi);
      imn = min(imn, (unsigned)imin3(Yi, Cri, Cbi)); imx = max(imx, (unsigned)imax3(Yi, Cri, Cbi));
      bgr2ycrcb_u8(r8b, r8g, r8r, Yj, Crj, Cbj);
      jmn = min(jmn, (unsigned)imin3(Yj, Crj, Cbj)); jmx = max(jmx, (unsigned)imax3(Yj, Crj, Cbj));
      out[c] = (uint32_t)Yi | ((uint32_t)Cri << 8) | ((uint32_t)Cbi << 16) | ((uint32_t)Yj << 24);
    }
    *reinterpret_cast<uint4*>(ycc + pp) = make_uint4(out[0], out[1], out[2], out[3]);
  }
  imn = warp_reduce_min_u32(imn); imx = warp_reduce_max_u32(imx);
  jmn = warp_reduce_min_u32(jmn); jmx = warp_reduce_max_u32(jmx);
  if ((threadIdx.x & 31) == 0) {
    FrameState& s = g.fs[f];
    atomicMin(&s.yi_min, imn); atomicMax(&s.yi_max, imx);
    atomicMin(&s.yj_min, jmn); atomicMax(&s.yj_max, jmx);
  }
}

constexpr uint32_t GP_S_NAN = 0xffffffffu;
__global__ void __launch_bounds__(256) stab_kernel(const FrameState* __restrict__ fs, uint32_t* __restrict__ stab) {
  int f = blockIdx.y, gy = blockIdx.x, j = threadIdx.x;
  const FrameState& s = fs[f];
  double yi_rng = (double)((int)s.yi_max - (int)s.yi_min), yj_rng = (double)((int)s.yj_max - (int)s.yj_min);
  double yi = (double)gy / yi_rng, yj = (double)j / yj_rng;
  double yi2 = 0.3 * (yi * yi);
  const double S = (yj * yi + yi2) / (yj * yj + yi2);
  stab[(size_t)f * 65536 + gy * 256 + j] = (S == S) ? __double2uint_rn(fmin(S, GP_S_PMAX) * GP_PSCALE) : GP_S_NAN;
}

__global__ void __launch_bounds__(256) splane_kernel(GfCommon g, int H, int Wp) {
  int f = blockIdx.y;
  size_t n_pp = (size_t)Wp * H;
  const FrameState& s = g.fs[f];
  const uint32_t a = s.yi_min, b = s.yj_min;
  const uint32_t ysub = a | (a << 8) | (a << 16) | (b << 24);
  const uint32_t* ycc = g.ycc + (size_t)f * n_pp;
  const uint32_t* stab = g.stab + (size_t)f * 65536;
  uint32_t* sp = g.splane + (size_t)f * n_pp;
  const size_t n_q = n_pp / 4;
  bool nan_seen = false;
  for (size_t qi = (size_t)blockIdx.x * 256 + threadIdx.x; qi < n_q; qi += (size_t)gridDim.x * 256) {
    uint4 yw = __ldg(reinterpret_cast<const uint4*>(ycc) + qi);
    uint32_t o[4];
#pragma unroll
    for (int c = 0; c < 4; c++) {
      uint32_t w = quad_get(yw, c);
      const bool pad = (w & 255u) < a || (w >> 24) < b;
      w -= ysub;
      const uint32_t S = pad ? 0u : __ldg(stab + (((w & 255u) << 8) | (w >> 24)));
      if (S == GP_S_NAN) nan_seen = true;
      o[c] = (S == GP_S_NAN) ? 0u : S;
    }
    reinterpret_cast<uint4*>(sp)[qi] = make_uint4(o[0], o[1], o[2], o[3]);
  }
  if (__any_sync(0xffffffffu, nan_seen) && (threadIdx.x & 31) == 0) atomicOr(&g.fs[f].nan_flag, 1u);
}

__global__ void __launch_bounds__(256, DZ_ELEMENTWISE_CTAS) final_kernel(GfCommon g, int W, int H, int Wp, uint8_t* __restrict__ dst, double* dbg_out, int32_t* __restrict__ flags) {
  __shared__ ExpShared sh;
  int f = blockIdx.y;
  size_t n_pp = (size_t)Wp * H;
  exp_shared_init(&sh, g.fs[f], (double)W * (double)H);
  const FrameState& s = g.fs[f];
  double omn = dunkey(s.omin_key), den = dunkey(s.omax_key) - omn;
  double scale = 255.0 / den;
  bool nan_frame = s.nan_flag != 0;
  if (flags && blockIdx.x == 0 && threadIdx.x == 0) flags[f] = nan_frame ? UWIP_FRAME_NAN : 0;
  const uint32_t* kq = g.kq + (size_t)f * n_pp;
  const float* J = g.J + (size_t)f * 2 * n_pp;
  const float* refS = g.refS + (size_t)f * n_pp;
  uint8_t* out = dst + (size_t)f * W * H * 3;
  const int qpr = Wp / 4;
  const size_t n_q = (size_t)qpr * H;
  const bool vec_ok = (W % 4 == 0) && ((reinterpret_cast<uintptr_t>(out) & 3) == 0);
  for (size_t qi = (size_t)blockIdx.x * 256 + threadIdx.x; qi < n_q; qi += (size_t)gridDim.x * 256) {
    int y = (int)(qi / qpr), x0 = (int)(qi - (size_t)y * qpr) * 4;
    size_t pp = (size_t)y * Wp + x0;
    uint4 kw = __ldg(reinterpret_cast<const uint4*>(kq + pp));
    float4 jb = __ldg(reinterpret_cast<const float4*>(J + pp)), jg = __ldg(reinterpret_cast<const float4*>(J + n_pp + pp));
    float4 qs = __ldg(reinterpret_cast<const float4*>(refS + pp));
    uint8_t b[12];
#pragma unroll
    for (int c = 0; c < 4; c++) {
      double rest[3];
      rest[0] = norm_j_fast(quad_get(jb, c), sh.fc, 0);
      rest[1] = norm_j_fast(quad_get(jg, c), sh.fc, 1);
      rest[2] = sh.rt.redN[(quad_get(kw, c) >> 16) & 255u];
      double q = (double)quad_get(qs, c);
#pragma unroll
      for (int ch = 0; ch < 3; ch++) {
        double v = (rest[ch] * q - omn) * scale;
        if (dbg_out && f == 0 && x0 + c < W) dbg_out[((size_t)y * W + x0 + c) * 3 + ch] = nan_frame ? __longlong_as_double(0x7ff8000000000000ll) : (rest[ch] * q - omn) / den;
        int bv = 0;
        if (!nan_frame && v == v && fabs(v) < 2.0e9) bv = min(max(__double2int_rn(v), 0), 255);
        b[c * 3 + ch] = (uint8_t)bv;
      }
    }
    uint8_t* o = out + ((size_t)y * W + x0) * 3;
    if (vec_ok) {
      uint32_t* o32 = reinterpret_cast<uint32_t*>(o);
      o32[0] = (uint32_t)b[0] | ((uint32_t)b[1] << 8) | ((uint32_t)b[2] << 16) | ((uint32_t)b[3] << 24);
      o32[1] = (uint32_t)b[4] | ((uint32_t)b[5] << 8) | ((uint32_t)b[6] << 16) | ((uint32_t)b[7] << 24);
      o32[2] = (uint32_t)b[8] | ((uint32_t)b[9] << 8) | ((uint32_t)b[10] << 16) | ((uint32_t)b[11] << 24);
    } else {
      for (int c = 0; c < 4 && x0 + c < W; c++) { o[c * 3] = b[c * 3]; o[c * 3 + 1] = b[c * 3 + 1]; o[c * 3 + 2] = b[c * 3 + 2]; }
    }
  }
}

int dehaze_strips(int w) {
  GfGeom g = gf_geometry(w, 4 * 40 + 2, 40);
  return cdiv(w, g.SW);
}
int dehaze_strips_narrow(int w) { return dehaze_gf1a_strips(w); }
int dehaze_sub_batch(const uwip_ctx* ctx, int n, int w, int cap) {
  cap = std::max(1, cap);
  if (n <= cap) return n;
  GfGeom g = gf_geometry(w, 4 * 40 + 2, 40);
  const long long sw = cdiv(w, g.SW), sn = dehaze_gf1a_strips(w), sms = std::max(1, ctx->sm_count);
  auto waves = [&](long long frames, long long strips) { return (double)((frames * strips + sms - 1) / sms) / (double)strips; };
  double best_cost = -1.0;
  int best = cap;
  for (int m = cap; m >= std::max(1, cap / 2); m--) {
    const int full = n / m, rem = n - full * m;
    double cost = full * (0.64 * waves(m, sw) + 0.36 * waves(m, sn)) + (rem ? 0.64 * waves(rem, sw) + 0.36 * waves(rem, sn) : 0.0);
    if (best_cost < 0.0 || cost < best_cost - 1e-9) { best_cost = cost; best = m; }
  }
  return best;
}

int dehaze_frames_dev(uwip_ctx* ctx, const uint8_t* d_src, uint8_t* d_dst, int n, int W, int H, const uwip_dehaze_params& p,
                      bool minmax_done, FrameState* fs, DehazeDebug* dbg, int32_t* d_flags) {
  UWIP_REQUIRE(ctx, n >= 1 && W >= 1 && H >= 1, "bad size");
  UWIP_REQUIRE(ctx, p.window >= 1 && p.window <= WK_MAXWIN, "window must be 1..33");
  UWIP_REQUIRE(ctx, p.radius >= 1 && p.radius <= GP_MAX_RADIUS, "radius must be 1..128");
  UWIP_REQUIRE(ctx, p.eps >= GP_MIN_EPS && p.tmin <= 1.0, "eps must be >= 1e-3 and tmin <= 1");
  UWIP_REQUIRE(ctx, (size_t)W * H < (1ull << 31), "frame too large");
  UWIP_REQUIRE(ctx, !dbg || n == 1, "stage outputs are single-frame");
  size_t n_px = (size_t)W * H;
  const int Wp = (W + 3) & ~3;
  size_t n_pp = (size_t)Wp * H;
  if (!minmax_done) {
    int want = (int)std::min<size_t>((n_px * 3 / 16 + 255) / 256, 1u << 16);
    int gxm = std::max(1, std::min(want, ctx->sm_count * 8 / n + 1));
    dim3 grid(gxm, n);
    UWIP_LAUNCH(ctx, "dz_minmax", minmax_kernel, grid, 256, 0, d_src, n_px * 3, fs);
  }
  uint32_t* d_kq = (uint32_t*)uwip_slot(ctx, SLOT_KQ, (size_t)n * n_pp * 4);
  uint8_t* d_mg = (uint8_t*)uwip_slot(ctx, SLOT_MPLANES, (size_t)n * n_pp);
  uint32_t* d_ycc = (uint32_t*)uwip_slot(ctx, SLOT_YCC, (size_t)n * n_pp * 4);
  uint32_t* d_stab = (uint32_t*)uwip_slot(ctx, SLOT_STAB, (size_t)n * 65536 * 4);
  uint32_t* d_sp = (uint32_t*)uwip_slot(ctx, SLOT_SPLANE, (size_t)n * n_pp * sizeof(uint32_t));
  dim3 gridw(cdiv(Wp, WK_TX), cdiv(H, WK_TY), n);
  dim3 gridf(cdiv(Wp, WF_TX), cdiv(H, WF_TY), n);
  int n_part = gridw.x * gridw.y, n_partf = gridf.x * gridf.y;
  ArgPartial* d_part = (ArgPartial*)uwip_slot(ctx, SLOT_PARTIALS, (size_t)n * std::max(n_part, n_partf) * sizeof(ArgPartial));
  int32_t* d_ab = (int32_t*)uwip_slot(ctx, SLOT_AB, (size_t)n * 8 * n_pp * sizeof(int32_t));
  float* d_J = (float*)uwip_slot(ctx, SLOT_J, (size_t)n * 2 * n_pp * sizeof(float));
  float* d_refS = (float*)uwip_slot(ctx, SLOT_REFS, (size_t)n * n_pp * sizeof(float));
  if (!d_kq || !d_mg || !d_ycc || !d_stab || !d_sp || !d_part || !d_ab || !d_J || !d_refS) return UWIP_ERR_NOMEM;
  {
    const int wmax = p.window, wmin = WK_TWIN;
    if (wmax != WK_TWIN) {
      int PL = std::max(wmax / 2, wmin / 2), PR = std::max(wmax - 1 - wmax / 2, wmin - 1 - wmin / 2);
      int RW = WK_TX + PL + PR, RH = WK_TY + PL + PR;
      size_t smem = ((size_t)2 * RW * RH + (size_t)3 * RH * WK_TX) * 4;
      UWIP_CUDA(ctx, uwip_func_smem(ctx, FUNC_WINDOW, window_kernel, smem));
      UWIP_LAUNCH(ctx, "dz_window", window_kernel, gridw, WK_THREADS, smem, d_src, W, H, Wp, wmax, fs, d_kq, d_mg, d_part);
      UWIP_LAUNCH(ctx, "dz_bglight", bglight_finish_kernel, n, 256, 0, d_src, W, H, d_part, n_part, fs, 1, 0);
    }
    size_t smemf = ((size_t)2 * WF_RH * WF_PP + (size_t)3 * WF_RH * WF_HP) * 4;
    UWIP_CUDA(ctx, uwip_func_smem(ctx, FUNC_WINDOW15, window15_kernel, smemf));
    UWIP_LAUNCH(ctx, "dz_window", window15_kernel, gridf, 256, smemf, d_src, W, H, Wp, fs, d_kq, d_mg, d_part);
    UWIP_LAUNCH(ctx, "dz_bglight", bglight_finish_kernel, n, 256, 0, d_src, W, H, d_part, n_partf, fs, wmax == WK_TWIN ? 1 : 0, 1);
  }
  if (dbg && dbg->stop_after == 1) return UWIP_OK;
  if (dbg && dbg->t_raw) {
    dim3 g2(cdiv(W, 256), H);
    UWIP_LAUNCH(ctx, "dz_traw", traw_kernel, g2, 256, 0, d_kq, d_mg, W, H, Wp, fs, dbg->t_raw);
  }
  if (dbg && dbg->stop_after == 2) return UWIP_OK;

  GfCommon gc;
  gc.kq = d_kq; gc.mg = d_mg; gc.ycc = d_ycc; gc.stab = d_stab; gc.splane = d_sp; gc.ab = d_ab; gc.J = d_J; gc.refS = d_refS; gc.fs = fs;
  gc.eps = p.eps; gc.tmin = p.tmin; gc.dbg_tref = dbg ? dbg->t_ref : nullptr;
  UWIP_CHECK(dehaze_gf1a_launch(ctx, gc, n, W, H, p.radius));
  UWIP_CHECK(gp_launch<PipGF1b>(ctx, "dz_gf1b", FUNC_GF1B, gc, n, W, H, p.radius));
  if (dbg && dbg->stop_after == 3) return UWIP_OK;
  int gx = std::max(1, std::min((int)((n_pp / 4 + 1023) / 1024), std::max(1, ctx->sm_count * 24 / n)));
  dim3 grid_e(gx, n);
  UWIP_LAUNCH(ctx, "dz_exposure_minmax", exposure_minmax_kernel, grid_e, 256, 0, gc, W, H, Wp, dbg ? dbg->restored : (double*)nullptr);
  if (dbg && dbg->stop_after == 4) return UWIP_OK;
  dim3 grid_s(256, n);
  UWIP_LAUNCH(ctx, "dz_stab", stab_kernel, grid_s, 256, 0, fs, d_stab);
  UWIP_LAUNCH(ctx, "dz_splane", splane_kernel, grid_e, 256, 0, gc, H, Wp);
  UWIP_CHECK(gp_launch<PipGF2a>(ctx, "dz_gf2a", FUNC_GF2A, gc, n, W, H, p.radius));
  UWIP_CHECK(gp_launch<PipGF2b>(ctx, "dz_gf2b", FUNC_GF2B, gc, n, W, H, p.radius));
  UWIP_LAUNCH(ctx, "dz_final", final_kernel, grid_e, 256, 0, gc, W, H, Wp, d_dst, dbg ? dbg->out : (double*)nullptr, d_flags);
  return UWIP_OK;
}

__global__ void __launch_bounds__(256) box_rows_kernel(const double* __restrict__ src, double* __restrict__ dst, int W, int H, int r) {
  const int x = blockIdx.x * 256 + threadIdx.x, y = blockIdx.y;
  if (x >= W) return;
  const double* row = src + (size_t)y * W;
  double s = 0.0;
  for (int k = max(x - r, 0); k <= min(x + r, W - 1); k++) s += row[k];
  dst[(size_t)y * W + x] = s;
}
__global__ void __launch_bounds__(256) box_cols_kernel(const double* __restrict__ src, double* __restrict__ dst, int W, int H, int r) {
  const int x = blockIdx.x * 256 + threadIdx.x, y = blockIdx.y;
  if (x >= W) return;
  double s = 0.0;
  for (int k = max(y - r, 0); k <= min(y + r, H - 1); k++) s += src[(size_t)k * W + x];
  dst[(size_t)y * W + x] = s;
}
int boxfilter_f64_dev(uwip_ctx* ctx, const double* d_src, double* d_tmp, double* d_dst, int W, int H, int r) {
  UWIP_REQUIRE(ctx, W >= 1 && H >= 1 && r >= 0, "bad size");
  dim3 grid(cdiv(W, 256), H);
  UWIP_LAUNCH(ctx, "box_rows", box_rows_kernel, grid, 256, 0, d_src, d_tmp, W, H, r);
  UWIP_LAUNCH(ctx, "box_cols", box_cols_kernel, grid, 256, 0, (const double*)d_tmp, d_dst, W, H, r);
  return UWIP_OK;
}

__global__ void __launch_bounds__(256) gfq_pack_kernel(const uint8_t* __restrict__ guide, const double* __restrict__ p, int W, int H, int Wp,
                                                       uint32_t* __restrict__ ycc, uint32_t* __restrict__ sp, FrameState* fs) {
  const int x = blockIdx.x * 256 + threadIdx.x, y = blockIdx.y;
  if (x >= Wp) return;
  uint32_t g = 0, P = 0;
  bool bad = false;
  if (x < W) {
    const uint8_t* q = guide + ((size_t)y * W + x) * 3;
    g = (uint32_t)q[0] | ((uint32_t)q[1] << 8) | ((uint32_t)q[2] << 16);
    const double v = p[(size_t)y * W + x];
    bad = !(v >= 0.0 && v <= GP_S_PMAX);
    P = bad ? 0u : __double2uint_rn(v * GP_PSCALE);
  }
  ycc[(size_t)y * Wp + x] = g;
  sp[(size_t)y * Wp + x] = P;
  if (bad) atomicOr(&fs[0].nan_flag, 2u);
}
__global__ void gfq_state_kernel(FrameState* fs, int range) {
  FrameState& s = fs[0];
  s.yi_min = 0; s.yi_max = (unsigned)range; s.yj_min = 0; s.yj_max = (unsigned)range;
  s.kmin = 0; s.kmax = (unsigned)range;
}
int guided_filter_u8_dev(uwip_ctx* ctx, const uint8_t* d_guide, const double* d_p, double* d_q, int W, int H, int range, int r, double eps,
                         FrameState* fs) {
  UWIP_REQUIRE(ctx, W >= 1 && H >= 1 && r >= 1 && r <= GP_MAX_RADIUS && range >= 1 && range <= 255 && eps >= GP_MIN_EPS, "bad argument");
  const int Wp = (W + 3) & ~3;
  const size_t n_pp = (size_t)Wp * H;
  uint32_t* d_ycc = (uint32_t*)uwip_slot(ctx, SLOT_YCC, n_pp * 4);
  uint32_t* d_sp = (uint32_t*)uwip_slot(ctx, SLOT_SPLANE, n_pp * 4);
  int32_t* d_ab = (int32_t*)uwip_slot(ctx, SLOT_AB, 8 * n_pp * 4);
  if (!d_ycc || !d_sp || !d_ab) return UWIP_ERR_NOMEM;
  UWIP_CHECK(frame_state_reset(ctx, fs, 1));
  UWIP_LAUNCH(ctx, "gfq_state", gfq_state_kernel, 1, 1, 0, fs, range);
  dim3 grid(cdiv(Wp, 256), H);
  UWIP_LAUNCH(ctx, "gfq_pack", gfq_pack_kernel, grid, 256, 0, d_guide, d_p, W, H, Wp, d_ycc, d_sp, fs);
  GfCommon gc;
  memset(&gc, 0, sizeof(gc));
  gc.ycc = d_ycc; gc.splane = d_sp; gc.ab = d_ab; gc.fs = fs; gc.eps = eps; gc.tmin = 0.0; gc.dbg_tref = d_q;
  UWIP_CHECK(gp_launch<PipGF2a>(ctx, "dz_gf2a", FUNC_GF2A, gc, 1, W, H, r));
  UWIP_CHECK(gp_launch<PipGFq>(ctx, "gfq_out", FUNC_GFQ, gc, 1, W, H, r));
  return UWIP_OK;
}
```

### uwimageproc_b200/csrc/gfmarch.cuh

```cuda
#pragma once
#include <algorithm>

#include "common.cuh"

__device__ __forceinline__ double u2d(uint32_t u) { return __uint2double_rn(u); }
__device__ __forceinline__ double rcp_fast(double x) {
  double r;
  asm("rcp.approx.ftz.f64 %0, %1;" : "=d"(r) : "d"(x));
  double e = fma(-x, r, 1.0);
  r = fma(r, e, r);
  e = fma(-x, r, 1.0);
  r = fma(r, e, r);
  return r;
}

__device__ __forceinline__ void cp_async16(void* smem, const void* g) {
  unsigned a = (unsigned)__cvta_generic_to_shared(smem);
  asm volatile("cp.async.cg.shared.global [%0], [%1], 16;" ::"r"(a), "l"(g) : "memory");
}
__device__ __forceinline__ void cp_async8(void* smem, const void* g) {
  asm volatile("cp.async.ca.shared.global [%0], [%1], 8;" ::"r"((unsigned)__cvta_generic_to_shared(smem)), "l"(g) : "memory");
}
__device__ __forceinline__ void cp_async_wait_2() { asm volatile("cp.async.wait_group 2;" ::: "memory"); }
__device__ __forceinline__ void cp_async4(void* smem, const void* g) {
  unsigned a = (unsigned)__cvta_generic_to_shared(smem);
  asm volatile("cp.async.ca.shared.global [%0], [%1], 4;" ::"r"(a), "l"(g) : "memory");
}
__device__ __forceinline__ void cp_async_commit() { asm volatile("cp.async.commit_group;" ::: "memory"); }
__device__ __forceinline__ void cp_async_wait_all() { asm volatile("cp.async.wait_group 0;" ::: "memory"); }
__device__ __forceinline__ void mbar_init(uint64_t* bar, unsigned count) {
  unsigned a = (unsigned)__cvta_generic_to_shared(bar);
  asm volatile("mbarrier.init.shared::cta.b64 [%0], %1;" ::"r"(a), "r"(count) : "memory");
}
__device__ __forceinline__ void mbar_arrive_expect_tx(uint64_t* bar, unsigned bytes) {
  unsigned a = (unsigned)__cvta_generic_to_shared(bar);
  asm volatile("mbarrier.arrive.expect_tx.shared::cta.b64 _, [%0], %1;" ::"r"(a), "r"(bytes) : "memory");
}

__device__ __forceinline__ void gf_build_M(const uint32_t* si, double N, double epsN2, double* M, double* Sd) {
  Sd[0] = u2d(si[0]); Sd[1] = u2d(si[1]); Sd[2] = u2d(si[2]);
  M[0] = fma(N, u2d(si[3]), -Sd[0] * Sd[0]) + epsN2;
  M[1] = fma(N, u2d(si[4]), -Sd[0] * Sd[1]);
  M[2] = fma(N, u2d(si[5]), -Sd[0] * Sd[2]);
  M[3] = fma(N, u2d(si[6]), -Sd[1] * Sd[1]) + epsN2;
  M[4] = fma(N, u2d(si[7]), -Sd[1] * Sd[2]);
  M[5] = fma(N, u2d(si[8]), -Sd[2] * Sd[2]) + epsN2;
}
__device__ __forceinline__ void gf_adjugate(const double* M, double* A, double& rdet) {
  A[0] = M[3] * M[5] - M[4] * M[4];
  A[1] = M[2] * M[4] - M[1] * M[5];
  A[2] = M[1] * M[4] - M[2] * M[3];
  A[3] = M[0] * M[5] - M[2] * M[2];
  A[4] = M[1] * M[2] - M[0] * M[4];
  A[5] = M[0] * M[3] - M[1] * M[1];
  double det = M[0] * A[0] + M[1] * A[1] + M[2] * A[2];
  rdet = rcp_fast(det);
}

struct GfCommon {
  const uint32_t* kq;
  const uint8_t* mg;
  uint32_t* ycc;
  const uint32_t* stab;
  uint32_t* splane;
  int32_t* ab;
  float* J;
  float* refS;
  FrameState* fs;
  double eps, tmin;
  double* dbg_tref;
};

constexpr int GP_MAX_RADIUS = 128;
constexpr double GP_MIN_EPS = 1e-3;

struct GfGeom {
  int W, H, Wp;
  int r;
  int HL;
  int SW;
  int NQ;
  int seg_h;
  int fast;
};

struct FrameConst {
  int kmin, range;
  double B[3], Bt[3];
  double jmin[2], jinv[2], jrcp[2];
  int yi_min, yi_rng, yj_min, yj_rng;
};

__device__ __forceinline__ void load_frame_const(const FrameState& s, FrameConst& c) {
  c.kmin = s.kmin;
  c.range = (int)s.kmax - (int)s.kmin;
  c.B[0] = s.B[0]; c.B[1] = s.B[1]; c.B[2] = s.B[2];
  c.Bt[0] = s.Bt[0]; c.Bt[1] = s.Bt[1]; c.Bt[2] = s.Bt[2];
  for (int k = 0; k < 2; k++) {
    double mn = dunkey(s.jmin_key[k]), mx = dunkey(s.jmax_key[k]);
    c.jmin[k] = mn;
    c.jinv[k] = mx - mn;
    c.jrcp[k] = 1.0 / (mx - mn);
  }
  c.yi_min = s.yi_min; c.yi_rng = (int)s.yi_max - (int)s.yi_min;
  c.yj_min = s.yj_min; c.yj_rng = (int)s.yj_max - (int)s.yj_min;
}

struct RedTables {
  double redN[256];
  uint8_t red8[256];
  uint8_t i8[256];
};
__device__ __forceinline__ int trunc_u8(double v) {
  if (!(v == v)) return 0;
  int i = (int)v;
  return i & 0xff;
}
static __device__ void build_red_tables(const FrameState& s, const FrameConst& fc, double n_px, RedTables* rt, int tid, int nthreads) {
  double range = (double)fc.range;
  double mean_b = ((double)s.jsum_fix[0] * (1.0 / 4294967296.0) / n_px - fc.jmin[0]) / fc.jinv[0];
  double mean_g = ((double)s.jsum_fix[1] * (1.0 / 4294967296.0) / n_px - fc.jmin[1]) / fc.jinv[1];
  double avgRr = 1.5 - mean_b - mean_g;
  double mean_r = ((double)s.rsum / n_px) / range;
  double coef = avgRr / mean_r;
  double ra = ((double)s.rmin / range) * coef, rb = ((double)s.rmax / range) * coef;
  double rmn = fmin(ra, rb), rmx = fmax(ra, rb);
  for (int k = tid; k < 256; k += nthreads) {
    double nk = (double)k / range;
    double v = (nk * coef - rmn) / (rmx - rmn);
    rt->redN[k] = v;
    rt->red8[k] = (uint8_t)trunc_u8(v * 255.0);
    rt->i8[k] = (uint8_t)trunc_u8(nk * 255.0);
  }
}

struct ExpShared {
  RedTables rt;
  FrameConst fc;
};
static __device__ void exp_shared_init(ExpShared* sh, const FrameState& s, double n_px) {
  if (threadIdx.x == 0) load_frame_const(s, sh->fc);
  __syncthreads();
  build_red_tables(s, sh->fc, n_px, &sh->rt, threadIdx.x, blockDim.x);
  __syncthreads();
}
__device__ __forceinline__ double norm_j(float j, const FrameConst& fc, int c) { return ((double)j - fc.jmin[c]) / fc.jinv[c]; }
__device__ __forceinline__ double norm_j_fast(float j, const FrameConst& fc, int c) { return ((double)j - fc.jmin[c]) * fc.jrcp[c]; }
__device__ __forceinline__ int restored_byte(float j, const FrameConst& fc, int c) {
  double v = norm_j_fast(j, fc, c) * 255.0;
  if (fabs(v - rint(v)) < 1.0e-9 || !(v == v)) v = norm_j(j, fc, c) * 255.0;
  return trunc_u8(v);
}

__device__ __forceinline__ long long warp_sum_i64(long long v) {
#pragma unroll
  for (int d = 16; d > 0; d >>= 1) v += __shfl_xor_sync(0xffffffffu, v, d);
  return v;
}
__device__ __forceinline__ float warp_min_f32(float v) {
#pragma unroll
  for (int d = 16; d > 0; d >>= 1) v = fminf(v, __shfl_xor_sync(0xffffffffu, v, d));
  return v;
}
__device__ __forceinline__ float warp_max_f32(float v) {
#pragma unroll
  for (int d = 16; d > 0; d >>= 1) v = fmaxf(v, __shfl_xor_sync(0xffffffffu, v, d));
  return v;
}
__device__ __forceinline__ double warp_min_f64(double v) {
#pragma unroll
  for (int d = 16; d > 0; d >>= 1) v = fmin(v, __shfl_xor_sync(0xffffffffu, v, d));
  return v;
}
__device__ __forceinline__ double warp_max_f64(double v) {
#pragma unroll
  for (int d = 16; d > 0; d >>= 1) v = fmax(v, __shfl_xor_sync(0xffffffffu, v, d));
  return v;
}

__device__ __forceinline__ uint32_t quad_get(const uint4& v, int c) { return c == 0 ? v.x : (c == 1 ? v.y : (c == 2 ? v.z : v.w)); }
__device__ __forceinline__ float quad_get(const float4& v, int c) { return c == 0 ? v.x : (c == 1 ? v.y : (c == 2 ? v.z : v.w)); }


template <int NP>
__device__ __forceinline__ int coef_chunk(int gq, int c, int j) {
  if (NP == 8) return (2 * c + j) ^ (gq & 7);
  return c ^ ((gq >> 1) & 3);
}

#include "gfpipe.cuh"

static GfGeom gf_geometry(int W, int H, int r) {
  GfGeom g;
  g.W = W; g.H = H; g.Wp = (W + 3) & ~3; g.r = r;
  g.HL = (r + 3) & ~3;
  int sw_max = std::min(4 * (GP_NTR - 1) - 2 * g.HL, GP_MAXSW);
  int strips = cdiv(W, sw_max);
  g.SW = (cdiv(W, strips) + 3) & ~3;
  g.NQ = 1 + (2 * g.HL + g.SW) / 4;
  g.seg_h = H;
  g.fast = (r % 4 == 0) ? 1 : 0;
  return g;
}

template <class P>
static int gp_launch(uwip_ctx* ctx, const char* tag, int func_id, const GfCommon& gc, int n, int W, int H, int r) {
  GfGeom gg = gf_geometry(W, H, r);
  int strips = cdiv(W, gg.SW);
  int slots = ctx->sm_count;
  int tasks = strips * n;
  int best = 1;
  double best_eff = 0.0;
  int max_segs = std::max(1, H / (4 * r + 2));
  for (int s = 1; s <= max_segs && s <= 64; s++) {
    int sh = cdiv(H, s), sc = cdiv(H, sh);
    double waves = (double)cdiv(tasks * sc, slots);
    double eff = ((double)tasks * sc / (waves * slots)) * ((double)sh / (double)(sh + 2 * r));
    if (eff > best_eff * 1.02) { best_eff = eff; best = s; }
  }
  gg.seg_h = cdiv(H, best);
  int segs = cdiv(H, gg.seg_h);
  static_assert(GpSmem<P>::bytes <= 227 * 1024, "shared memory");
  size_t smem = GpSmem<P>::bytes;
  UWIP_CUDA(ctx, uwip_func_smem(ctx, func_id, gp_kernel<P>, smem));
  dim3 grid(strips, segs, n);
  UWIP_LAUNCH(ctx, tag, gp_kernel<P>, grid, GP_THREADS, smem, gc, gg);
  return UWIP_OK;
}
```

### uwimageproc_b200/csrc/gfpipe.cuh

```cuda
#pragma once

#ifndef GP_NARROW
#define GP_NARROW 0
#endif
constexpr int GP_AUX_REGS = 88;
constexpr int GP_GF1A_ACC_REGS = GP_NARROW ? 176 : 152;
constexpr int GP_GF2A_ACC_REGS = GP_NARROW ? 168 : 144;
constexpr int GP_B_ACC_REGS = GP_NARROW ? 128 : 136;

constexpr int GP_NT = GP_NARROW ? 128 : 160;
constexpr int GP_NTR = GP_NT < 152 ? GP_NT : 152;
constexpr int GP_NAUX = GP_NARROW ? 4 : 3;
constexpr int GP_SOLVE_THREADS = 256;
constexpr int GP_ACC_THREADS = GP_NT + 32 * GP_NAUX;
constexpr int GP_THREADS = GP_ACC_THREADS + GP_SOLVE_THREADS;
constexpr int GP_MAXSW = 2 * GP_SOLVE_THREADS;
constexpr int GP_NSEG = 8, GP_SEGQ = 20;
constexpr int GP_GP = GP_NSEG * GP_SEGQ;
constexpr int GP_SEG_PAD = 2;
constexpr int GP_SEGD = GP_SEGQ + GP_SEG_PAD;
constexpr int GP_GPD = GP_NSEG * GP_SEGD;
__device__ __forceinline__ int gp_dpos(int t) { return t + GP_SEG_PAD * (t / GP_SEGQ); }
static_assert(GP_GP >= GP_NT, "thread layout");

// ... 545 lines not shown
    const Shared* sh; int Wp;
    const uint32_t* kq; const uint8_t* mg;
    __device__ __forceinline__ void init(const GfCommon& g, int f, Shared* s, const GfGeom& gg) {
      sh = s; Wp = gg.Wp;
      const size_t n_pp = (size_t)gg.Wp * gg.H;
      kq = g.kq + (size_t)f * n_pp;
      mg = g.mg + (size_t)f * n_pp;
    }
    __device__ __forceinline__ void stage_issue(unsigned char* st, int s, int y, int gx, int t) const {
      const size_t o = (size_t)y * Wp + gx;
      cp_async16(st + ((size_t)s * GP_NT + t) * 16, kq + o);
      cp_async4(st + (size_t)4 * GP_NT * 16 + ((size_t)s * GP_NT + t) * 4, mg + o);
    }
    __device__ __forceinline__ void stage_read(const unsigned char* st, int s, Raw& r, int t) const {
      r.k = *reinterpret_cast<const uint4*>(st + ((size_t)s * GP_NT + t) * 16);
      r.m = *reinterpret_cast<const uint32_t*>(st + (size_t)4 * GP_NT * 16 + ((size_t)s * GP_NT + t) * 4);
    }
    template <int SIGN, bool FULL>
    __device__ __forceinline__ void accum(const Raw& r, unsigned cmask, uint32_t (&Vi)[4][NI], double (&Vl)[4][ND]) const {
#pragma unroll
      for (int c = 0; c < 4; c++) {
        const uint32_t w = quad_get(r.k, c);
        const int kb = (int)(w & 255u), kg = (int)((w >> 8) & 255u), kr = (int)((w >> 16) & 255u);
        const uint32_t mb = w >> 24, mgv = (r.m >> (8 * c)) & 255u;
        const int sb = SIGN > 0 ? kb : -kb, sg = SIGN > 0 ? kg : -kg, sr = SIGN > 0 ? kr : -kr;
        Vi[c][0] += (uint32_t)sb; Vi[c][1] += (uint32_t)sg; Vi[c][2] += (uint32_t)sr;
        Vi[c][3] += (uint32_t)(sb * kb); Vi[c][4] += (uint32_t)(sb * kg); Vi[c][5] += (uint32_t)(sb * kr);
        Vi[c][6] += (uint32_t)(sg * kg); Vi[c][7] += (uint32_t)(sg * kr); Vi[c][8] += (uint32_t)(sr * kr);
        if (FULL || (cmask & (1u << c))) {
          const double pb = sh->pT[0][mb], pg = sh->pT[1][mgv];
          Vl[c][0] += SIGN > 0 ? pb : -pb; Vl[c][1] += SIGN > 0 ? pg : -pg;
          const double db = (double)sb, dg = (double)sg, dr = (double)sr;
          Vl[c][2] = fma(db, pb, Vl[c][2]); Vl[c][3] = fma(dg, pb, Vl[c][3]); Vl[c][4] = fma(dr, pb, Vl[c][4]);
          Vl[c][5] = fma(db, pg, Vl[c][5]); Vl[c][6] = fma(dg, pg, Vl[c][6]); Vl[c][7] = fma(dr, pg, Vl[c][7]);
        }
      }
    }
  };
  struct Solve {
    const Shared* sh; int Wp; int32_t* ab;
    GpInvN cinv;
    __device__ __forceinline__ void init(const GfCommon& g, int f, Shared* s, const GfGeom& gg) {
      sh = s; Wp = gg.Wp;
      ab = g.ab + (size_t)f * 8 * (size_t)gg.Wp * gg.H;
    }
    __device__ __forceinline__ void row_prefetch(int, int, unsigned char*) {}
    __device__ __forceinline__ void row_pickup(const unsigned char*) {}
    __device__ __forceinline__ void column(int cc, int y, int x, int Ncnt, const uint32_t* si, const double* sd, bool valid) {
      const double N = u2d((uint32_t)Ncnt), invN = cinv.get(cc, Ncnt);
      double M[6], Sd[3], A[6], rdet;
      gf_build_M(si, N, sh->epsN_k * N * N, M, Sd);
      gf_adjugate(M, A, rdet);
      const double pinv = sh->pinv;
      rdet *= pinv;
      double a0[3], b0, a1[3], b1;
      const int gq = x >> 2, c = x & 3;
      int4* blk = reinterpret_cast<int4*>(ab) + ((size_t)y * (Wp >> 2) + gq) * 8;
      gp_solve_rhs(A, rdet, Sd, N, invN, pinv, sd[0], sd + 2, a0, b0);
      gp_solve_rhs(A, rdet, Sd, N, invN, pinv, sd[1], sd + 5, a1, b1);
      if (valid) {
        blk[coef_chunk<8>(gq, c, 0)] = coef_pack_fix(a0, b0, sh->cs.sa, sh->cs.sb);
        blk[coef_chunk<8>(gq, c, 1)] = coef_pack_fix(a1, b1, sh->cs.sa, sh->cs.sb);
      }
    }
    __device__ __forceinline__ void store_pair(int, int, bool) {}
    __device__ __forceinline__ void finish() {}
  };
};

struct PipGF2a {
  static constexpr int NI = 9, ND = 4, NSTAGE = 3, ACC_REGS = GP_GF2A_ACC_REGS, SOLVE_REGS = GP_SOLVE_REGS_FOR(GP_GF2A_ACC_REGS);
  static constexpr bool PLANE_READER = false;
  static constexpr int IN_BYTES = 4 * GP_NT * 32;
  static constexpr int SOLVE_FIELDS = 0;
  struct Shared { FrameConst fc; double epsN_k, pinv; CoefScale cs; };
  static __device__ void init_shared(const GfCommon& g, int f, Shared* sh, const GfGeom& gg) {
    if (threadIdx.x == 0) {
      load_frame_const(g.fs[f], sh->fc);
      const double rng = (double)sh->fc.yi_rng;
      sh->epsN_k = g.eps * rng * rng;
      sh->cs = coef_scale(g.eps, rng);
      sh->pinv = GP_PINV;
    }
    __syncthreads();
  }
  struct Acc {
    struct Raw { uint4 y; uint4 s; };
    int Wp; const uint32_t* ycc; const uint32_t* sp;
    uint32_t ysub;
    __device__ __forceinline__ void init(const GfCommon& g, int f, Shared* s, const GfGeom& gg) {
      Wp = gg.Wp;
      const size_t n_pp = (size_t)gg.Wp * gg.H;
      ycc = g.ycc + (size_t)f * n_pp;
      sp = g.splane + (size_t)f * n_pp;
      const uint32_t a = (uint32_t)s->fc.yi_min, b = (uint32_t)s->fc.yj_min;
      ysub = a | (a << 8) | (a << 16) | (b << 24);
    }
    __device__ __forceinline__ void stage_issue(unsigned char* st, int s, int y, int gx, int t) const {
      const size_t o = (size_t)y * Wp + gx;
      cp_async16(st + ((size_t)s * GP_NT + t) * 32, ycc + o);
      cp_async16(st + ((size_t)s * GP_NT + t) * 32 + 16, sp + o);
    }
    __device__ __forceinline__ void stage_read(const unsigned char* st, int s, Raw& r, int t) const {
      r.y = *reinterpret_cast<const uint4*>(st + ((size_t)s * GP_NT + t) * 32);
      r.s = *reinterpret_cast<const uint4*>(st + ((size_t)s * GP_NT + t) * 32 + 16);
    }
    template <int SIGN, bool FULL>
    __device__ __forceinline__ void accum(const Raw& r, unsigned cmask, uint32_t (&Vi)[4][NI], double (&Vl)[4][ND]) const {
#pragma unroll
      for (int c = 0; c < 4; c++) {
        if (FULL || (cmask & (1u << c))) {
          const uint32_t w = quad_get(r.y, c) - ysub;
          const int g0 = (int)(w & 255u), g1 = (int)((w >> 8) & 255u), g2 = (int)((w >> 16) & 255u);
          const double S = u2d(quad_get(r.s, c));
          const int s0 = SIGN > 0 ? g0 : -g0, s1 = SIGN > 0 ? g1 : -g1, s2 = SIGN > 0 ? g2 : -g2;
          Vi[c][0] += (uint32_t)s0; Vi[c][1] += (uint32_t)s1; Vi[c][2] += (uint32_t)s2;
          Vi[c][3] += (uint32_t)(s0 * g0); Vi[c][4] += (uint32_t)(s0 * g1); Vi[c][5] += (uint32_t)(s0 * g2);
          Vi[c][6] += (uint32_t)(s1 * g1); Vi[c][7] += (uint32_t)(s1 * g2); Vi[c][8] += (uint32_t)(s2 * g2);
          Vl[c][0] += SIGN > 0 ? S : -S;
          Vl[c][1] = fma((double)s0, S, Vl[c][1]); Vl[c][2] = fma((double)s1, S, Vl[c][2]); Vl[c][3] = fma((double)s2, S, Vl[c][3]);
        }
      }
    }
  };
  struct Solve {
    const Shared* sh; int Wp; int32_t* ab;
    GpInvN cinv;
    __device__ __forceinline__ void init(const GfCommon& g, int f, Shared* s, const GfGeom& gg) {
      sh = s; Wp = gg.Wp;
      ab = g.ab + (size_t)f * 8 * (size_t)gg.Wp * gg.H;
    }
    __device__ __forceinline__ void row_prefetch(int, int, unsigned char*) {}
    __device__ __forceinline__ void row_pickup(const unsigned char*) {}
    __device__ __forceinline__ void column(int cc, int y, int x, int Ncnt, const uint32_t* si, const double* sd, bool valid) {
      const double N = u2d((uint32_t)Ncnt), invN = cinv.get(cc, Ncnt);
      double M[6], Sd[3], A[6], rdet, a[3], b;
      gf_build_M(si, N, sh->epsN_k * N * N, M, Sd);
      gf_adjugate(M, A, rdet);
      const double pinv = sh->pinv;
      rdet *= pinv;
      gp_solve_rhs(A, rdet, Sd, N, invN, pinv, sd[0], sd + 1, a, b);
      const int gq = x >> 2;
      int4* blk = reinterpret_cast<int4*>(ab) + ((size_t)y * (Wp >> 2) + gq) * 4;
      if (valid) blk[coef_chunk<4>(gq, x & 3, 0)] = coef_pack_fix(a, b, sh->cs.sa, sh->cs.sb);
    }
    __device__ __forceinline__ void store_pair(int, int, bool) {}
    __device__ __forceinline__ void finish() {}
  };
};

__device__ __forceinline__ int4 lds128i(unsigned addr) {
  int4 v;
  asm volatile("ld.shared.v4.s32 {%0,%1,%2,%3}, [%4];" : "=r"(v.x), "=r"(v.y), "=r"(v.z), "=r"(v.w) : "r"(addr));
  return v;
}
template <int NP, bool ENTER, bool LEAVE, bool FULL>
__device__ __forceinline__ void gp_accum_coef_case(const int4* be_p, const int4* bl_p, int gq, unsigned cmask, double (&Vl)[4][NP]) {
  const unsigned swz = (unsigned)coef_chunk<NP>(gq, 0, 0) << 4;
  const unsigned be = (unsigned)__cvta_generic_to_shared(be_p) + swz;
  const unsigned bl = (unsigned)__cvta_generic_to_shared(bl_p) + swz;
#pragma unroll
  for (int c = 0; c < 4; c++) {
#pragma unroll
    for (int j = 0; j < NP / 4; j++) {
      const unsigned q16 = (unsigned)(NP == 8 ? 2 * c + j : c) << 4;
      int4 e = make_int4(0, 0, 0, 0), l = make_int4(0, 0, 0, 0);
      if (ENTER) e = lds128i(be ^ q16);
      if (LEAVE) l = lds128i(bl ^ q16);
      if (FULL || (cmask & (1u << c))) {
        Vl[c][4 * j + 0] += (double)(e.x - l.x); Vl[c][4 * j + 1] += (double)(e.y - l.y);
        Vl[c][4 * j + 2] += (double)(e.z - l.z); Vl[c][4 * j + 3] += (double)(e.w - l.w);
      }
    }
  }
}
template <int NP>
__device__ __forceinline__ void gp_accum_coef(const int4* be, const int4* bl, int gq, bool enter, bool leave, unsigned cmask, double (&Vl)[4][NP]) {
  if (enter && leave) {
    if (cmask == 0xfu) gp_accum_coef_case<NP, true, true, true>(be, bl, gq, cmask, Vl);
    else gp_accum_coef_case<NP, true, true, false>(be, bl, gq, cmask, Vl);
  } else if (enter) {
    gp_accum_coef_case<NP, true, false, false>(be, bl, gq, cmask, Vl);
  } else if (leave) {
    gp_accum_coef_case<NP, false, true, false>(be, bl, gq, cmask, Vl);
  }
}

struct PipGF1b {
  static constexpr float L2_FRAC = 0.5f;
  static constexpr int NI = 0, ND = 8, NP = 8, NSTAGE = 2, NRING = 3, ACC_REGS = GP_B_ACC_REGS, SOLVE_REGS = GP_SOLVE_REGS_FOR(GP_B_ACC_REGS);
  static constexpr bool PLANE_READER = true;
  static constexpr int IN_BYTES = NRING * 2 * GP_NTR * NP * 16;
  static constexpr int SOLVE_FIELDS = 0;
  struct Shared {
    double inv_range;
    FrameConst fc;
    CoefScale cs;
  };
  static __device__ void init_shared(const GfCommon& g, int f, Shared* sh, const GfGeom&) {
    if (threadIdx.x == 0) {
      load_frame_const(g.fs[f], sh->fc); sh->cs = coef_scale(g.eps, (double)sh->fc.range);
      sh->inv_range = 1.0 / (double)sh->fc.range;
    }
    __syncthreads();
  }
  static __device__ __forceinline__ const void* coef_rows(const GfCommon& g, int f, const GfGeom& gg) {
    return g.ab + (size_t)f * 8 * (size_t)gg.Wp * gg.H;
  }
  struct Acc {
    __device__ __forceinline__ void init(const GfCommon&, int, Shared*, const GfGeom&) {}
    __device__ __forceinline__ void accum_staged(const int4* be, const int4* bl, int gq, bool enter, bool leave, unsigned cmask, double (&Vl)[4][ND]) const {
      gp_accum_coef<NP>(be, bl, gq, enter, leave, cmask, Vl);
    }
  };
  struct Solve {
    const Shared* sh; GfCommon g; int W, Wp, H, f;
    const uint32_t* kq; float* J;
    float jmn[2], jmx[2];
    long long jsum[2];
    unsigned cnt, rmn, rmx, rsum, nanf;
    uint2 knext, kcur;
    float o[2][2];
    double* dbg;
    __device__ __forceinline__ void init(const GfCommon& gc, int frame, Shared* s, const GfGeom& gg) {
      g = gc; sh = s; W = gg.W; Wp = gg.Wp; H = gg.H; f = frame;
      dbg = (frame == 0) ? gc.dbg_tref : nullptr;
      const size_t n_pp = (size_t)Wp * H;
      kq = g.kq + (size_t)f * n_pp;
      J = g.J + (size_t)f * 2 * n_pp;
      jmn[0] = jmn[1] = __int_as_float(0x7f800000); jmx[0] = jmx[1] = -__int_as_float(0x7f800000);
      jsum[0] = jsum[1] = 0;
      cnt = 0; rmn = 255; rmx = 0; rsum = 0; nanf = 0;
      o[0][0] = o[0][1] = o[1][0] = o[1][1] = 0.f;
    }
    __device__ __forceinline__ void row_prefetch(int y, int x, unsigned char*) { knext = __ldg(reinterpret_cast<const uint2*>(kq + (size_t)y * Wp + x)); }
    __device__ __forceinline__ void row_pickup(const unsigned char*) { kcur = knext; }
    __device__ __forceinline__ void column(int cc, int y, int x, int Ncnt, const uint32_t*, const double* sd, bool valid) {
      const double invN = rcp_fast(u2d((uint32_t)Ncnt));
      const uint32_t w = cc ? kcur.y : kcur.x;
      const uint32_t k[3] = {w & 255u, (w >> 8) & 255u, (w >> 16) & 255u};
      const double kd[3] = {u2d(k[0]), u2d(k[1]), u2d(k[2])};
      const double isa = sh->cs.isa * invN, isb = sh->cs.isb * invN;
#pragma unroll
      for (int c = 0; c < 2; c++) {
        const double* s = sd + 4 * c;
        const double q = (s[0] * kd[0] + s[1] * kd[1] + s[2] * kd[2]) * isa + s[3] * isb;
        if (dbg && valid) dbg[(size_t)c * W * H + (size_t)y * W + x] = q;
        const double Bc = sh->fc.B[c];
        const double Jv = (kd[c] * sh->inv_range - Bc) * rcp_fast(q) + Bc;
        float Jf = (float)Jv;
        o[cc][c] = Jf;
        if (valid) {
          if (!(fabsf(Jf) < 262144.0f)) { nanf |= 1u; Jf = 0.f; }
          jmn[c] = fminf(jmn[c], Jf);
          jmx[c] = fmaxf(jmx[c], Jf);
          jsum[c] += __double_as_longlong(fma((double)Jf, 4294967296.0, 6755399441055744.0));
        }
      }
      if (valid) {
        cnt++;
        rmn = min(rmn, k[2]); rmx = max(rmx, k[2]); rsum += k[2];
      }
    }
    __device__ __forceinline__ void store_pair(int y, int x, bool second) {
      const size_t n_pp = (size_t)Wp * H, pp = (size_t)y * Wp + x;
      if (!second) { o[1][0] = 0.f; o[1][1] = 0.f; }
      *reinterpret_cast<float2*>(J + pp) = make_float2(o[0][0], o[1][0]);
      *reinterpret_cast<float2*>(J + n_pp + pp) = make_float2(o[0][1], o[1][1]);
    }
    __device__ __forceinline__ void finish() {
      FrameState& s = g.fs[f];
      for (int c = 0; c < 2; c++) {
        float a = warp_min_f32(jmn[c]), b = warp_max_f32(jmx[c]);
        long long sm = warp_sum_i64(jsum[c] - (long long)cnt * __double_as_longlong(6755399441055744.0));
        if ((threadIdx.x & 31) == 0) {
          if (a <= b) {
            atomicMin(&s.jmin_key[c], dkey((double)a));
            atomicMax(&s.jmax_key[c], dkey((double)b));
          }
          atomicAdd((unsigned long long*)&s.jsum_fix[c], (unsigned long long)sm);
        }
      }
      unsigned a = warp_reduce_min_u32(rmn), b = warp_reduce_max_u32(rmx);
      unsigned rs = __reduce_add_sync(0xffffffffu, rsum);
      unsigned nf = __reduce_or_sync(0xffffffffu, nanf);
      if ((threadIdx.x & 31) == 0) {
        atomicMin(&s.rmin, a);
        atomicMax(&s.rmax, b);
        atomicAdd(&s.rsum, (unsigned long long)rs);
        if (nf) atomicOr(&s.nan_flag, nf);
      }
    }
  };
};

struct PipGF2b {
  static constexpr float L2_FRAC = 1.0f;
  static constexpr int NI = 0, ND = 4, NP = 4, NSTAGE = 3, NRING = 4, ACC_REGS = GP_B_ACC_REGS, SOLVE_REGS = GP_SOLVE_REGS_FOR(GP_B_ACC_REGS);
  static constexpr bool PLANE_READER = true;
  static constexpr int IN_BYTES = NRING * 2 * GP_NTR * NP * 16;
  static constexpr int SOLVE_FIELDS = 4;
  struct Shared { ExpShared e; CoefScale cs; };
  static __device__ void init_shared(const GfCommon& g, int f, Shared* sh, const GfGeom& gg) {
    exp_shared_init(&sh->e, g.fs[f], (double)gg.W * (double)gg.H);
    if (threadIdx.x == 0) sh->cs = coef_scale(g.eps, (double)sh->e.fc.yi_rng);
    __syncthreads();
  }
  static __device__ __forceinline__ const void* coef_rows(const GfCommon& g, int f, const GfGeom& gg) {
    return g.ab + (size_t)f * 8 * (size_t)gg.Wp * gg.H;
  }
  struct Acc {
    __device__ __forceinline__ void init(const GfCommon&, int, Shared*, const GfGeom&) {}
    __device__ __forceinline__ void accum_staged(const int4* be, const int4* bl, int gq, bool enter, bool leave, unsigned cmask, double (&Vl)[4][ND]) const {
      gp_accum_coef<NP>(be, bl, gq, enter, leave, cmask, Vl);
    }
  };
  struct Solve {
    const Shared* sh; GfCommon g; int Wp, H, f;
    const uint32_t* kq; const uint32_t* ycc; const float* J; float* refS;
    double omn, omx; unsigned nanf;
    uint2 kc, yc; float2 jbc, jgc;
    float o[2];
    __device__ __forceinline__ void init(const GfCommon& gc, int frame, Shared* s, const GfGeom& gg) {
      g = gc; sh = s; Wp = gg.Wp; H = gg.H; f = frame;
      const size_t n_pp = (size_t)Wp * H;
      kq = g.kq + (size_t)f * n_pp;
      ycc = g.ycc + (size_t)f * n_pp;
      J = g.J + (size_t)f * 2 * n_pp;
      refS = g.refS + (size_t)f * n_pp;
      omn = __longlong_as_double(0x7ff0000000000000ll); omx = -omn; nanf = 0;
      o[0] = o[1] = 0.f;
    }
    static constexpr int FLD = GP_SOLVE_THREADS * 8;
    __device__ __forceinline__ void row_prefetch(int y, int x, unsigned char* st) {
      const size_t n_pp = (size_t)Wp * H, p = (size_t)y * Wp + x;
      cp_async8(st, kq + p);
      cp_async8(st + FLD, ycc + p);
      cp_async8(st + 2 * FLD, J + p);
      cp_async8(st + 3 * FLD, J + n_pp + p);
    }
    __device__ __forceinline__ void row_pickup(const unsigned char* st) {
      kc = *reinterpret_cast<const uint2*>(st); yc = *reinterpret_cast<const uint2*>(st + FLD);
      jbc = *reinterpret_cast<const float2*>(st + 2 * FLD); jgc = *reinterpret_cast<const float2*>(st + 3 * FLD);
    }
    __device__ __forceinline__ void column(int cc, int, int, int Ncnt, const uint32_t*, const double* sd, bool valid) {
      const double invN = rcp_fast(u2d((uint32_t)Ncnt));
      const uint32_t yw = cc ? yc.y : yc.x;
      const uint32_t ymin = (uint32_t)sh->e.fc.yi_min;
      const double g0 = u2d((yw & 255u) - ymin), g1 = u2d(((yw >> 8) & 255u) - ymin), g2 = u2d(((yw >> 16) & 255u) - ymin);
      const double q = ((sd[0] * g0 + sd[1] * g1 + sd[2] * g2) * sh->cs.isa + sd[3] * sh->cs.isb) * invN;
      const float qf = (float)q;
      o[cc] = qf;
      const double qr = (double)qf;
      const double rb = norm_j_fast(cc ? jbc.y : jbc.x, sh->e.fc, 0), rg = norm_j_fast(cc ? jgc.y : jgc.x, sh->e.fc, 1);
      const double rr = sh->e.rt.redN[((cc ? kc.y : kc.x) >> 16) & 255u];
      const double o0 = rb * qr, o1 = rg * qr, o2 = rr * qr;
      const double os = (o0 + o1) + o2;
      if (!valid) {}
      else if (!(os == os) || fabs(os) > 1.0e300) { nanf = 1u; }
      else {
        double lo = o0 < o1 ? o0 : o1, hi = o0 < o1 ? o1 : o0;
        lo = o2 < lo ? o2 : lo; hi = o2 > hi ? o2 : hi;
        omn = lo < omn ? lo : omn;
        omx = hi > omx ? hi : omx;
      }
    }
    __device__ __forceinline__ void store_pair(int y, int x, bool second) {
      if (!second) o[1] = 0.f;
      *reinterpret_cast<float2*>(refS + (size_t)y * Wp + x) = make_float2(o[0], o[1]);
    }
    __device__ __forceinline__ void finish() {
      const double a = warp_min_f64(omn), b = warp_max_f64(omx);
      const unsigned nf = __reduce_or_sync(0xffffffffu, nanf);
      if ((threadIdx.x & 31) == 0) {
        if (a <= b) {
          atomicMin(&g.fs[f].omin_key, dkey(a));
          atomicMax(&g.fs[f].omax_key, dkey(b));
        }
        if (nf) atomicOr(&g.fs[f].nan_flag, 1u);
      }
    }
  };
};

struct PipGFq {
  static constexpr float L2_FRAC = 1.0f;
  static constexpr int NI = 0, ND = 4, NP = 4, NSTAGE = 3, NRING = 4, ACC_REGS = GP_B_ACC_REGS, SOLVE_REGS = GP_SOLVE_REGS_FOR(GP_B_ACC_REGS);
  static constexpr bool PLANE_READER = true;
  static constexpr int IN_BYTES = NRING * 2 * GP_NTR * NP * 16;
  static constexpr int SOLVE_FIELDS = 1;
  struct Shared { FrameConst fc; CoefScale cs; };
  static __device__ void init_shared(const GfCommon& g, int f, Shared* sh, const GfGeom&) {
    if (threadIdx.x == 0) { load_frame_const(g.fs[f], sh->fc); sh->cs = coef_scale(g.eps, (double)sh->fc.yi_rng); }
    __syncthreads();
  }
  static __device__ __forceinline__ const void* coef_rows(const GfCommon& g, int f, const GfGeom& gg) {
    return g.ab + (size_t)f * 8 * (size_t)gg.Wp * gg.H;
  }
  struct Acc {
    __device__ __forceinline__ void init(const GfCommon&, int, Shared*, const GfGeom&) {}
    __device__ __forceinline__ void accum_staged(const int4* be, const int4* bl, int gq, bool enter, bool leave, unsigned cmask, double (&Vl)[4][ND]) const {
      gp_accum_coef<NP>(be, bl, gq, enter, leave, cmask, Vl);
    }
  };
  struct Solve {
    const Shared* sh; int W, Wp;
    const uint32_t* ycc; double* q_out;
    uint2 yc;
    __device__ __forceinline__ void init(const GfCommon& g, int f, Shared* s, const GfGeom& gg) {
      sh = s; W = gg.W; Wp = gg.Wp;
      ycc = g.ycc + (size_t)f * (size_t)gg.Wp * gg.H;
      q_out = g.dbg_tref + (size_t)f * (size_t)gg.W * gg.H;
    }
    __device__ __forceinline__ void row_prefetch(int y, int x, unsigned char* st) { cp_async8(st, ycc + (size_t)y * Wp + x); }
    __device__ __forceinline__ void row_pickup(const unsigned char* st) { yc = *reinterpret_cast<const uint2*>(st); }
    __device__ __forceinline__ void column(int cc, int y, int x, int Ncnt, const uint32_t*, const double* sd, bool valid) {
      const double invN = rcp_fast(u2d((uint32_t)Ncnt));
      const uint32_t yw = cc ? yc.y : yc.x;
      const uint32_t ymin = (uint32_t)sh->fc.yi_min;
      const double g0 = u2d((yw & 255u) - ymin), g1 = u2d(((yw >> 8) & 255u) - ymin), g2 = u2d(((yw >> 16) & 255u) - ymin);
      if (valid) q_out[(size_t)y * W + x] = ((sd[0] * g0 + sd[1] * g1 + sd[2] * g2) * sh->cs.isa + sd[3] * sh->cs.isb) * invN;
    }
    __device__ __forceinline__ void store_pair(int, int, bool) {}
    __device__ __forceinline__ void finish() {}
  };
};
```

Before: 1253.

## Replace per-pixel f64 exposure byte computation with float threshold table lookup

A new per-frame kernel precomputes the red/intensity tables once and builds float threshold tables, found by binary search, that map each J value to its restored byte. The exposure min/max kernel then uses a float guess plus a two-compare correction instead of double-precision normalization. A fallback exact kernel handles frames whose table fails validation or when debug output is requested. This removes redundant per-block table construction and most f64 arithmetic from a hot elementwise pass, at the cost of one extra small kernel, an extra (mostly early-exit) launch, and a new test entry point.

```diff
diff --git a/include/uwip.h b/include/uwip.h
--- a/include/uwip.h
+++ b/include/uwip.h
@@ -126,6 +126,8 @@
                        double* out_f64);
 int uwip_bgdehaze_bgr8_dev(uwip_ctx* ctx, const uint8_t* d_src, uint8_t* d_dst, int n_frames,
                            int width, int height, const uwip_dehaze_params* p);
+int uwip_exposure_bytes_check(uwip_ctx* ctx, const double jmin[2], const double jmax[2], const float* J, int n, float* T,
+                              int* use_table, uint8_t* via_table, uint8_t* direct);
 
 typedef struct uwip_chain_params {
   char channels[16];
diff --git a/uwimageproc_b200/_lib.py b/uwimageproc_b200/_lib.py
--- a/uwimageproc_b200/_lib.py
+++ b/uwimageproc_b200/_lib.py
@@ -77,6 +77,7 @@
     "uwip_rc_correction_bgr8": (_i, [_P, _u8p, _sz, _i, _i, C.POINTER(DehazeParams), _P]),
     "uwip_bgdehaze_bgr8": (_i, [_P, _u8p, _sz, _u8p, _sz, _i, _i, C.POINTER(DehazeParams), _P]),
     "uwip_bgdehaze_bgr8_dev": (_i, [_P, _u8p, _u8p, _i, _i, _i, C.POINTER(DehazeParams)]),
+    "uwip_exposure_bytes_check": (_i, [_P, C.POINTER(_d), C.POINTER(_d), _P, _i, _P, C.POINTER(_i), _P, _P]),
     "uwip_chain_bgr8_dev": (_i, [_P, _u8p, _u8p, _i, _i, _i, C.POINTER(ChainParams)]),
     "uwip_chain_bgr8_auto_dev": (_i, [_P, _u8p, _u8p, _i, _i, _i, C.POINTER(ChainParams), _i, _P, _P]),
     "uwip_chain_bgr8": (_i, [_P, _u8p, _u8p, _i, _i, _i, C.POINTER(ChainParams)]),
diff --git a/uwimageproc_b200/csrc/cabi.cu b/uwimageproc_b200/csrc/cabi.cu
--- a/uwimageproc_b200/csrc/cabi.cu
+++ b/uwimageproc_b200/csrc/cabi.cu
@@ -581,6 +581,29 @@
   return UWIP_OK;
 }
 
+int uwip_exposure_bytes_check(uwip_ctx* ctx, const double jmin[2], const double jmax[2], const float* J, int n, float* T,
+                              int* use_table, uint8_t* via_table, uint8_t* direct) {
+  CTX_GUARD(ctx);
+  UWIP_REQUIRE(ctx, jmin && jmax && T && use_table && n >= 0 && (n == 0 || (J && via_table && direct)), "bad argument");
+  const size_t nj = 2 * (size_t)n;
+  uint8_t* d = (uint8_t*)uwip_slot(ctx, SLOT_F64OUT, nj * 6 + 2064);
+  if (!d) return UWIP_ERR_NOMEM;
+  float* d_T = (float*)d;
+  float* d_J = (float*)(d + 2048);
+  uint8_t* d_tab = d + 2048 + nj * 4;
+  if (n > 0) UWIP_CUDA(ctx, cudaMemcpyAsync(d_J, J, nj * 4, cudaMemcpyHostToDevice, ctx->stream));
+  int* d_use = (int*)(d_tab + 2 * nj);
+  UWIP_CHECK(dehaze_exposure_bytes_dev(ctx, jmin, jmax, d_J, n, d_T, d_tab, d_tab + nj, d_use));
+  UWIP_CUDA(ctx, cudaMemcpyAsync(T, d_T, 2048, cudaMemcpyDeviceToHost, ctx->stream));
+  UWIP_CUDA(ctx, cudaMemcpyAsync(use_table, d_use, sizeof(int), cudaMemcpyDeviceToHost, ctx->stream));
+  if (n > 0) {
+    UWIP_CUDA(ctx, cudaMemcpyAsync(via_table, d_tab, nj, cudaMemcpyDeviceToHost, ctx->stream));
+    UWIP_CUDA(ctx, cudaMemcpyAsync(direct, d_tab + nj, nj, cudaMemcpyDeviceToHost, ctx->stream));
+  }
+  UWIP_CUDA(ctx, cudaStreamSynchronize(ctx->stream));
+  return UWIP_OK;
+}
+
 static int32_t* flags_get(uwip_ctx* ctx, int n) {
   int32_t* f = (int32_t*)uwip_slot(ctx, SLOT_FLAGS, sizeof(int32_t) * (size_t)n);
   ctx->flags_n = f ? n : 0;
@@ -665,7 +688,8 @@
       {SLOT_TMP_FRAME, fbytes * m}, {SLOT_HIST, (size_t)m * 256 * 4}, {SLOT_LUT, (size_t)m * 256 * 4},
       {SLOT_TILEHIST, ntile * 256 * 4}, {SLOT_TILELUT, ntile * 256 + 16}, {SLOT_MISC, 256},
       {SLOT_KQ, m * n_pp * 4}, {SLOT_MPLANES, m * n_pp}, {SLOT_YCC, m * n_pp * 4}, {SLOT_STAB, (size_t)m * 65536 * 8},
-      {SLOT_SPLANE, m * n_pp * 4}, {SLOT_AB, m * n_pp * 32}, {SLOT_J, m * n_pp * 8}, {SLOT_REFS, m * n_pp * 4}};
+      {SLOT_SPLANE, m * n_pp * 4}, {SLOT_AB, m * n_pp * 32}, {SLOT_J, m * n_pp * 8}, {SLOT_REFS, m * n_pp * 4},
+      {SLOT_EXPTAB, m * DZ_EXPTAB_BYTES}};
   for (const auto& e : want)
     if (!uwip_slot(ctx, e.slot, e.bytes)) return UWIP_ERR_NOMEM;
   return UWIP_OK;
diff --git a/uwimageproc_b200/csrc/common.cuh b/uwimageproc_b200/csrc/common.cuh
--- a/uwimageproc_b200/csrc/common.cuh
+++ b/uwimageproc_b200/csrc/common.cuh
@@ -25,7 +25,7 @@
   std::vector<cudaEvent_t> ev_pool;
   cudaStream_t s_in = nullptr, s_out = nullptr;
   std::string err;
-  static const int kSlots = 32;
+  static const int kSlots = 33;
   void* slot_ptr[kSlots] = {};
   size_t slot_bytes[kSlots] = {};
   void* pinned = nullptr;
@@ -79,7 +79,9 @@
   SLOT_AUTO,
   SLOT_AUTO_BSCL,
   SLOT_JPEGENC,
-};
+  SLOT_EXPTAB,
+};
+constexpr size_t DZ_EXPTAB_BYTES = 4672;
 
 const char* uwip_set_err(uwip_ctx* ctx, const char* fmt, ...);
 void* uwip_slot(uwip_ctx* ctx, int slot, size_t bytes);
@@ -345,6 +347,8 @@
 FrameState* frame_state_get(uwip_ctx* ctx, int n);
 int boxfilter_f64_dev(uwip_ctx* ctx, const double* d_src, double* d_tmp, double* d_dst, int w, int h, int r);
 int guided_filter_u8_dev(uwip_ctx* ctx, const uint8_t* d_guide, const double* d_p, double* d_q, int w, int h, int range, int r, double eps, FrameState* fs);
+int dehaze_exposure_bytes_dev(uwip_ctx* ctx, const double jmin[2], const double jmax[2], const float* d_J, int n, float* d_T,
+                              uint8_t* d_via_table, uint8_t* d_direct, int* d_use_table);
 
 int jpeg_info(uwip_ctx* ctx, const uint8_t* data, size_t len, int* w, int* h);
 int jpeg_decode_dev(uwip_ctx* ctx, const uint8_t* data, size_t len, uint8_t* d_bgr, int w, int h);
diff --git a/uwimageproc_b200/csrc/dehaze.cu b/uwimageproc_b200/csrc/dehaze.cu
--- a/uwimageproc_b200/csrc/dehaze.cu
+++ b/uwimageproc_b200/csrc/dehaze.cu
@@ -464,44 +464,118 @@
   t_raw[(size_t)W * H + pix] = 1.0 - ((double)mg / range) / s.Bt[1];
 }
 
+__device__ __forceinline__ int fkey(float v) { const int i = __float_as_int(v); return i >= 0 ? i : i ^ 0x7fffffff; }
+__device__ __forceinline__ float funkey(int k) { return __int_as_float(k >= 0 ? k : k ^ 0x7fffffff); }
+
+__global__ void __launch_bounds__(256) exptab_kernel(const FrameState* __restrict__ fs, ExpTables* __restrict__ et, double n_px) {
+  __shared__ FrameConst fc;
+  __shared__ int s_bad;
+  const int f = blockIdx.x, v = threadIdx.x;
+  const FrameState& s = fs[f];
+  ExpTables& t = et[f];
+  if (v == 0) { load_frame_const(s, fc); s_bad = 0; }
+  __syncthreads();
+  {
+    double range = (double)fc.range;
+    double mean_b = ((double)s.jsum_fix[0] * (1.0 / 4294967296.0) / n_px - fc.jmin[0]) / fc.jinv[0];
+    double mean_g = ((double)s.jsum_fix[1] * (1.0 / 4294967296.0) / n_px - fc.jmin[1]) / fc.jinv[1];
+    double avgRr = 1.5 - mean_b - mean_g;
+    double mean_r = ((double)s.rsum / n_px) / range;
+    double coef = avgRr / mean_r;
+    double ra = ((double)s.rmin / range) * coef, rb = ((double)s.rmax / range) * coef;
+    double rmn = fmin(ra, rb), rmx = fmax(ra, rb);
+    double nk = (double)v / range;
+    double rv = (nk * coef - rmn) / (rmx - rmn);
+    t.redN[v] = rv;
+    t.b.red8[v] = (uint8_t)trunc_u8(rv * 255.0);
+    t.b.i8[v] = (uint8_t)trunc_u8(nk * 255.0);
+  }
+  const float inf = __int_as_float(0x7f800000);
+  for (int c = 0; c < 2; c++) {
+    const float lo = (float)dunkey(s.jmin_key[c]), hi = (float)dunkey(s.jmax_key[c]);
+    const float scale = __fdiv_rn(255.f, __fsub_rn(hi, lo));
+    const bool range_ok = lo <= hi;
+    float T = -inf;
+    if (v > 0) {
+      if (!range_ok || restored_byte(hi, fc, c) < v) T = inf;
+      else if (restored_byte(lo, fc, c) >= v) T = lo;
+      else {
+        long long a = fkey(lo), b = fkey(hi);
+        while (b - a > 1) {
+          const long long m = a + ((b - a) >> 1);
+          if (restored_byte(funkey((int)m), fc, c) >= v) b = m; else a = m;
+        }
+        T = funkey((int)b);
+      }
+    }
+    t.b.T[c][v] = T;
+    if (v < EXP_TN - 256) t.b.T[c][256 + v] = inf;
+    bool bad = !range_ok;
+    if (!bad) {
+      auto off = [&](float j) { const int d = exp_guess(j, lo, scale) - restored_byte(j, fc, c); return d < -1 || d > 1; };
+      if (v > 0 && T > lo && T <= hi) bad = off(T) || off(funkey(fkey(T) - 1));
+      if (v == 0) bad = off(lo) || off(hi);
+    }
+    if (bad) s_bad = 1;
+    if (v == 0) { t.b.lo[c] = lo; t.b.scale[c] = scale; }
+  }
+  __syncthreads();
+  if (v == 0) t.b.use_table = (s_bad || (s.nan_flag & 1u)) ? 0 : 1;
+  if (v < 3) t.b.pad[v] = 0;
+}
+
 constexpr int DZ_ELEMENTWISE_CTAS = 4;
-__global__ void __launch_bounds__(256, DZ_ELEMENTWISE_CTAS) exposure_minmax_kernel(GfCommon g, int W, int H, int Wp, double* dbg_restored) {
-  __shared__ ExpShared sh;
-  int f = blockIdx.y;
-  size_t n_pp = (size_t)Wp * H;
-  exp_shared_init(&sh, g.fs[f], (double)W * (double)H);
+template <bool TABLE>
+__global__ void __launch_bounds__(256, TABLE ? DZ_ELEMENTWISE_CTAS : 2) exposure_minmax_kernel(GfCommon g, int W, int H, int Wp, double* dbg_restored) {
+  __shared__ __align__(16) ExpBytes sb;
+  __shared__ FrameConst fc;
+  const int f = blockIdx.y;
+  if (TABLE != (g.et[f].b.use_table && !dbg_restored)) return;
+  {
+    const uint4* src = reinterpret_cast<const uint4*>(&g.et[f].b);
+    for (int i = threadIdx.x; i < (int)(sizeof(ExpBytes) / 16); i += 256) reinterpret_cast<uint4*>(&sb)[i] = __ldg(src + i);
+    if (!TABLE && threadIdx.x == 0) load_frame_const(g.fs[f], fc);
+  }
+  __syncthreads();
+  const float lo0 = sb.lo[0], sc0 = sb.scale[0], lo1 = sb.lo[1], sc1 = sb.scale[1];
+  const size_t n_pp = (size_t)Wp * H;
   const uint32_t* kq = g.kq + (size_t)f * n_pp;
   const float* J = g.J + (size_t)f * 2 * n_pp;
   uint32_t* ycc = g.ycc + (size_t)f * n_pp;
   unsigned imn = 255, imx = 0, jmn = 255, jmx = 0;
-  const int qpr = Wp / 4;
-  const size_t n_q = (size_t)qpr * H;
-  for (size_t qi = (size_t)blockIdx.x * 256 + threadIdx.x; qi < n_q; qi += (size_t)gridDim.x * 256) {
-    int y = (int)(qi / qpr), x0 = (int)(qi - (size_t)y * qpr) * 4;
-    size_t pp = (size_t)y * Wp + x0;
-    uint4 kw = __ldg(reinterpret_cast<const uint4*>(kq + pp));
-    float4 jb = __ldg(reinterpret_cast<const float4*>(J + pp)), jg = __ldg(reinterpret_cast<const float4*>(J + n_pp + pp));
+  const unsigned qpr = (unsigned)Wp / 4, n_q = qpr * (unsigned)H;
+  for (unsigned qi = blockIdx.x * 256 + threadIdx.x; qi < n_q; qi += gridDim.x * 256) {
+    const int y = (int)(qi / qpr), x0 = (int)(qi - (unsigned)y * qpr) * 4;
+    const uint4 kw = __ldg(reinterpret_cast<const uint4*>(kq) + qi);
+    const float4 jb = __ldg(reinterpret_cast<const float4*>(J) + qi), jg = __ldg(reinterpret_cast<const float4*>(J + n_pp) + qi);
     uint32_t out[4];
 #pragma unroll
     for (int c = 0; c < 4; c++) {
       out[c] = 0;
       if (x0 + c >= W) continue;
-      uint32_t w = quad_get(kw, c);
-      uint32_t kb = w & 255u, kg = (w >> 8) & 255u, kr = (w >> 16) & 255u;
-      int r8b = restored_byte(quad_get(jb, c), sh.fc, 0), r8g = restored_byte(quad_get(jg, c), sh.fc, 1), r8r = sh.rt.red8[kr];
-      if (dbg_restored && f == 0) {
-        size_t pix = (size_t)y * W + x0 + c;
-        dbg_restored[pix * 3] = norm_j(quad_get(jb, c), sh.fc, 0); dbg_restored[pix * 3 + 1] = norm_j(quad_get(jg, c), sh.fc, 1);
-        dbg_restored[pix * 3 + 2] = sh.rt.redN[kr];
+      const uint32_t w = quad_get(kw, c);
+      const uint32_t kb = w & 255u, kg = (w >> 8) & 255u, kr = (w >> 16) & 255u;
+      const float vb = quad_get(jb, c), vg = quad_get(jg, c);
+      int r8b, r8g;
+      if (TABLE) {
+        r8b = exp_table_byte(vb, sb.T[0], lo0, sc0); r8g = exp_table_byte(vg, sb.T[1], lo1, sc1);
+      } else {
+        r8b = restored_byte(vb, fc, 0); r8g = restored_byte(vg, fc, 1);
+        if (dbg_restored && f == 0) {
+          const size_t pix = (size_t)y * W + x0 + c;
+          dbg_restored[pix * 3] = norm_j(vb, fc, 0); dbg_restored[pix * 3 + 1] = norm_j(vg, fc, 1);
+          dbg_restored[pix * 3 + 2] = g.et[f].redN[kr];
+        }
       }
+      const int r8r = sb.red8[kr];
       int Yi, Cri, Cbi, Yj, Crj, Cbj;
-      bgr2ycrcb_u8(sh.rt.i8[kb], sh.rt.i8[kg], sh.rt.i8[kr], Yi, Cri, Cbi);
+      bgr2ycrcb_u8(sb.i8[kb], sb.i8[kg], sb.i8[kr], Yi, Cri, Cbi);
       imn = min(imn, (unsigned)imin3(Yi, Cri, Cbi)); imx = max(imx, (unsigned)imax3(Yi, Cri, Cbi));
       bgr2ycrcb_u8(r8b, r8g, r8r, Yj, Crj, Cbj);
       jmn = min(jmn, (unsigned)imin3(Yj, Crj, Cbj)); jmx = max(jmx, (unsigned)imax3(Yj, Crj, Cbj));
       out[c] = (uint32_t)Yi | ((uint32_t)Cri << 8) | ((uint32_t)Cbi << 16) | ((uint32_t)Yj << 24);
     }
-    *reinterpret_cast<uint4*>(ycc + pp) = make_uint4(out[0], out[1], out[2], out[3]);
+    reinterpret_cast<uint4*>(ycc)[qi] = make_uint4(out[0], out[1], out[2], out[3]);
   }
   imn = warp_reduce_min_u32(imn); imx = warp_reduce_max_u32(imx);
   jmn = warp_reduce_min_u32(jmn); jmx = warp_reduce_max_u32(jmx);
@@ -555,7 +629,7 @@
   __shared__ ExpShared sh;
   int f = blockIdx.y;
   size_t n_pp = (size_t)Wp * H;
-  exp_shared_init(&sh, g.fs[f], (double)W * (double)H);
+  exp_shared_init(&sh, g.fs[f], g.et[f]);
   const FrameState& s = g.fs[f];
   double omn = dunkey(s.omin_key), den = dunkey(s.omax_key) - omn;
   double scale = 255.0 / den;
@@ -580,7 +654,7 @@
       double rest[3];
       rest[0] = norm_j_fast(quad_get(jb, c), sh.fc, 0);
       rest[1] = norm_j_fast(quad_get(jg, c), sh.fc, 1);
-      rest[2] = sh.rt.redN[(quad_get(kw, c) >> 16) & 255u];
+      rest[2] = sh.redN[(quad_get(kw, c) >> 16) & 255u];
       double q = (double)quad_get(qs, c);
 #pragma unroll
       for (int ch = 0; ch < 3; ch++) {
@@ -653,7 +727,8 @@
   int32_t* d_ab = (int32_t*)uwip_slot(ctx, SLOT_AB, (size_t)n * 8 * n_pp * sizeof(int32_t));
   float* d_J = (float*)uwip_slot(ctx, SLOT_J, (size_t)n * 2 * n_pp * sizeof(float));
   float* d_refS = (float*)uwip_slot(ctx, SLOT_REFS, (size_t)n * n_pp * sizeof(float));
-  if (!d_kq || !d_mg || !d_ycc || !d_stab || !d_sp || !d_part || !d_ab || !d_J || !d_refS) return UWIP_ERR_NOMEM;
+  ExpTables* d_et = (ExpTables*)uwip_slot(ctx, SLOT_EXPTAB, (size_t)n * sizeof(ExpTables));
+  if (!d_kq || !d_mg || !d_ycc || !d_stab || !d_sp || !d_part || !d_ab || !d_J || !d_refS || !d_et) return UWIP_ERR_NOMEM;
   {
     const int wmax = p.window, wmin = WK_TWIN;
     if (wmax != WK_TWIN) {
@@ -677,14 +752,17 @@
   if (dbg && dbg->stop_after == 2) return UWIP_OK;
 
   GfCommon gc;
-  gc.kq = d_kq; gc.mg = d_mg; gc.ycc = d_ycc; gc.stab = d_stab; gc.splane = d_sp; gc.ab = d_ab; gc.J = d_J; gc.refS = d_refS; gc.fs = fs;
+  gc.kq = d_kq; gc.mg = d_mg; gc.ycc = d_ycc; gc.stab = d_stab; gc.splane = d_sp; gc.ab = d_ab; gc.J = d_J; gc.refS = d_refS; gc.et = d_et; gc.fs = fs;
   gc.eps = p.eps; gc.tmin = p.tmin; gc.dbg_tref = dbg ? dbg->t_ref : nullptr;
   UWIP_CHECK(dehaze_gf1a_launch(ctx, gc, n, W, H, p.radius));
   UWIP_CHECK(gp_launch<PipGF1b>(ctx, "dz_gf1b", FUNC_GF1B, gc, n, W, H, p.radius));
   if (dbg && dbg->stop_after == 3) return UWIP_OK;
+  UWIP_LAUNCH(ctx, "dz_exptab", exptab_kernel, n, 256, 0, fs, d_et, (double)W * (double)H);
   int gx = std::max(1, std::min((int)((n_pp / 4 + 1023) / 1024), std::max(1, ctx->sm_count * 24 / n)));
   dim3 grid_e(gx, n);
-  UWIP_LAUNCH(ctx, "dz_exposure_minmax", exposure_minmax_kernel, grid_e, 256, 0, gc, W, H, Wp, dbg ? dbg->restored : (double*)nullptr);
+  double* dbg_restored = dbg ? dbg->restored : nullptr;
+  UWIP_LAUNCH(ctx, "dz_exposure_minmax", exposure_minmax_kernel<true>, grid_e, 256, 0, gc, W, H, Wp, dbg_restored);
+  UWIP_LAUNCH(ctx, "dz_exposure_exact", exposure_minmax_kernel<false>, grid_e, 256, 0, gc, W, H, Wp, dbg_restored);
   if (dbg && dbg->stop_after == 4) return UWIP_OK;
   dim3 grid_s(256, n);
   UWIP_LAUNCH(ctx, "dz_stab", stab_kernel, grid_s, 256, 0, fs, d_stab);
@@ -692,6 +770,36 @@
   UWIP_CHECK(gp_launch<PipGF2a>(ctx, "dz_gf2a", FUNC_GF2A, gc, n, W, H, p.radius));
   UWIP_CHECK(gp_launch<PipGF2b>(ctx, "dz_gf2b", FUNC_GF2B, gc, n, W, H, p.radius));
   UWIP_LAUNCH(ctx, "dz_final", final_kernel, grid_e, 256, 0, gc, W, H, Wp, d_dst, dbg ? dbg->out : (double*)nullptr, d_flags);
+  return UWIP_OK;
+}
+
+__global__ void expbytes_kernel(const ExpTables* __restrict__ et, const FrameState* __restrict__ fs, const float* __restrict__ J, int n,
+                                uint8_t* __restrict__ via_table, uint8_t* __restrict__ direct) {
+  __shared__ FrameConst fc;
+  if (threadIdx.x == 0) load_frame_const(fs[0], fc);
+  __syncthreads();
+  const ExpBytes& b = et->b;
+  for (int i = blockIdx.x * blockDim.x + threadIdx.x; i < 2 * n; i += gridDim.x * blockDim.x) {
+    const int c = i < n ? 0 : 1;
+    via_table[i] = (uint8_t)exp_table_byte(J[i], b.T[c], b.lo[c], b.scale[c]);
+    direct[i] = (uint8_t)restored_byte(J[i], fc, c);
+  }
+}
+int dehaze_exposure_bytes_dev(uwip_ctx* ctx, const double jmin[2], const double jmax[2], const float* d_J, int n, float* d_T,
+                              uint8_t* d_via_table, uint8_t* d_direct, int* d_use_table) {
+  FrameState* fs = frame_state_get(ctx, 1);
+  ExpTables* d_et = (ExpTables*)uwip_slot(ctx, SLOT_EXPTAB, sizeof(ExpTables));
+  if (!fs || !d_et) return UWIP_ERR_NOMEM;
+  FrameState* hs = (FrameState*)ctx->pinned;
+  memset(hs, 0, sizeof(FrameState));
+  hs->kmin = 0; hs->kmax = 255; hs->rmin = 0; hs->rmax = 255; hs->rsum = 128;
+  for (int c = 0; c < 2; c++) { hs->jmin_key[c] = dkey(jmin[c]); hs->jmax_key[c] = dkey(jmax[c]); }
+  UWIP_CUDA(ctx, cudaMemcpyAsync(fs, hs, sizeof(FrameState), cudaMemcpyHostToDevice, ctx->stream));
+  UWIP_LAUNCH(ctx, "dz_exptab", exptab_kernel, 1, 256, 0, fs, d_et, 1.0);
+  if (n > 0) UWIP_LAUNCH(ctx, "dz_expbytes", expbytes_kernel, std::min(cdiv(2 * n, 256), 1024), 256, 0, d_et, fs, d_J, n, d_via_table, d_direct);
+  for (int c = 0; c < 2; c++)
+    UWIP_CUDA(ctx, cudaMemcpyAsync(d_T + 256 * c, d_et->b.T[c], 256 * sizeof(float), cudaMemcpyDeviceToDevice, ctx->stream));
+  UWIP_CUDA(ctx, cudaMemcpyAsync(d_use_table, &d_et->b.use_table, sizeof(int), cudaMemcpyDeviceToDevice, ctx->stream));
   return UWIP_OK;
 }
 
diff --git a/uwimageproc_b200/csrc/gfmarch.cuh b/uwimageproc_b200/csrc/gfmarch.cuh
--- a/uwimageproc_b200/csrc/gfmarch.cuh
+++ b/uwimageproc_b200/csrc/gfmarch.cuh
@@ -57,6 +57,7 @@
   rdet = rcp_fast(det);
 }
 
+struct ExpTables;
 struct GfCommon {
   const uint32_t* kq;
   const uint8_t* mg;
@@ -66,6 +67,7 @@
   int32_t* ab;
   float* J;
   float* refS;
+  ExpTables* et;
   FrameState* fs;
   double eps, tmin;
   double* dbg_tref;
@@ -106,43 +108,10 @@
   c.yj_min = s.yj_min; c.yj_rng = (int)s.yj_max - (int)s.yj_min;
 }
 
-struct RedTables {
-  double redN[256];
-  uint8_t red8[256];
-  uint8_t i8[256];
-};
 __device__ __forceinline__ int trunc_u8(double v) {
   if (!(v == v)) return 0;
   int i = (int)v;
   return i & 0xff;
-}
-static __device__ void build_red_tables(const FrameState& s, const FrameConst& fc, double n_px, RedTables* rt, int tid, int nthreads) {
-  double range = (double)fc.range;
-  double mean_b = ((double)s.jsum_fix[0] * (1.0 / 4294967296.0) / n_px - fc.jmin[0]) / fc.jinv[0];
-  double mean_g = ((double)s.jsum_fix[1] * (1.0 / 4294967296.0) / n_px - fc.jmin[1]) / fc.jinv[1];
-  double avgRr = 1.5 - mean_b - mean_g;
-  double mean_r = ((double)s.rsum / n_px) / range;
-  double coef = avgRr / mean_r;
-  double ra = ((double)s.rmin / range) * coef, rb = ((double)s.rmax / range) * coef;
-  double rmn = fmin(ra, rb), rmx = fmax(ra, rb);
-  for (int k = tid; k < 256; k += nthreads) {
-    double nk = (double)k / range;
-    double v = (nk * coef - rmn) / (rmx - rmn);
-    rt->redN[k] = v;
-    rt->red8[k] = (uint8_t)trunc_u8(v * 255.0);
-    rt->i8[k] = (uint8_t)trunc_u8(nk * 255.0);
-  }
-}
-
-struct ExpShared {
-  RedTables rt;
-  FrameConst fc;
-};
-static __device__ void exp_shared_init(ExpShared* sh, const FrameState& s, double n_px) {
-  if (threadIdx.x == 0) load_frame_const(s, sh->fc);
-  __syncthreads();
-  build_red_tables(s, sh->fc, n_px, &sh->rt, threadIdx.x, blockDim.x);
-  __syncthreads();
 }
 __device__ __forceinline__ double norm_j(float j, const FrameConst& fc, int c) { return ((double)j - fc.jmin[c]) / fc.jinv[c]; }
 __device__ __forceinline__ double norm_j_fast(float j, const FrameConst& fc, int c) { return ((double)j - fc.jmin[c]) * fc.jrcp[c]; }
@@ -150,6 +119,39 @@
   double v = norm_j_fast(j, fc, c) * 255.0;
   if (fabs(v - rint(v)) < 1.0e-9 || !(v == v)) v = norm_j(j, fc, c) * 255.0;
   return trunc_u8(v);
+}
+
+constexpr int EXP_TN = 260;
+struct ExpBytes {
+  float T[2][EXP_TN];
+  uint8_t red8[256];
+  uint8_t i8[256];
+  float lo[2], scale[2];
+  int use_table;
+  int pad[3];
+};
+struct ExpTables {
+  ExpBytes b;
+  double redN[256];
+};
+static_assert(sizeof(ExpBytes) % 16 == 0 && sizeof(ExpTables) == DZ_EXPTAB_BYTES, "16-byte copies; slot size");
+
+__device__ __forceinline__ int exp_guess(float j, float lo, float scale) {
+  return (int)fminf(fmaxf(__fmul_rn(__fsub_rn(j, lo), scale), 0.f), 255.f);
+}
+__device__ __forceinline__ int exp_table_byte(float j, const float* T, float lo, float scale) {
+  const int g = exp_guess(j, lo, scale);
+  return g - (j < T[g] ? 1 : 0) + (j >= T[g + 1] ? 1 : 0);
+}
+
+struct ExpShared {
+  double redN[256];
+  FrameConst fc;
+};
+static __device__ void exp_shared_init(ExpShared* sh, const FrameState& s, const ExpTables& et) {
+  if (threadIdx.x == 0) load_frame_const(s, sh->fc);
+  for (int k = threadIdx.x; k < 256; k += blockDim.x) sh->redN[k] = et.redN[k];
+  __syncthreads();
 }
 
 __device__ __forceinline__ long long warp_sum_i64(long long v) {
diff --git a/uwimageproc_b200/csrc/gfpipe.cuh b/uwimageproc_b200/csrc/gfpipe.cuh
--- a/uwimageproc_b200/csrc/gfpipe.cuh
+++ b/uwimageproc_b200/csrc/gfpipe.cuh
@@ -871,7 +871,7 @@
   static constexpr int SOLVE_FIELDS = 4;
   struct Shared { ExpShared e; CoefScale cs; };
   static __device__ void init_shared(const GfCommon& g, int f, Shared* sh, const GfGeom& gg) {
-    exp_shared_init(&sh->e, g.fs[f], (double)gg.W * (double)gg.H);
+    exp_shared_init(&sh->e, g.fs[f], g.et[f]);
     if (threadIdx.x == 0) sh->cs = coef_scale(g.eps, (double)sh->e.fc.yi_rng);
     __syncthreads();
   }
@@ -922,7 +922,7 @@
       o[cc] = qf;
       const double qr = (double)qf;
       const double rb = norm_j_fast(cc ? jbc.y : jbc.x, sh->e.fc, 0), rg = norm_j_fast(cc ? jgc.y : jgc.x, sh->e.fc, 1);
-      const double rr = sh->e.rt.redN[((cc ? kc.y : kc.x) >> 16) & 255u];
+      const double rr = sh->e.redN[((cc ? kc.y : kc.x) >> 16) & 255u];
       const double o0 = rb * qr, o1 = rg * qr, o2 = rr * qr;
       const double os = (o0 + o1) + o2;
       if (!valid) {}
```

Result: no change. 1264, median of 6 (+0.9%).
